# Yun-960/Pytorch-Distributed-Template

Hardware: AMD Instinct MI355X
Metric: images/sec (whole node) ResNet-50 synthetic 3x224x224 at 1/2/4/8 MI355X (higher is better)
Workload: dtype bf16; 1 GPU; model=resnet50, global_batch=2048, per_gpu_batch=2048, image_size=224, parallelism=dp1, backend=native, optimizer=SGD(lr=0.1, momentum=0.9, wd=5e-5), dist_backend=nccl, ddp=True, ddp_impl=BucketedDDP, device=cuda, hip_graph=False, ddp_fallback_copies=0

## Files before the change

### csrc/conv3x3_halo.hip

```cpp
#include "conv_nt_kernel.h"

namespace pdt_nt {
namespace {

constexpr int HBM = 224;
constexpr int HWM = 2;
constexpr int PMAX = 384;
constexpr int PBYTES = PMAX * 128;
constexpr int ZBYTES = 1024;

template <int BN, int NTH, int SGN, int BNB>
__global__ void __launch_bounds__(NTH, 1) conv3x3_halo_kernel(NTParams p, int rs_log2, int ntm, int ntn, int ncc) {
  constexpr int WN = NTH / 64 / HWM;
  constexpr int MI = HBM / (HWM * 16);
  constexpr int NI = BN / (WN * 16);
  constexpr int SB = BN * 128;
  constexpr int LB = BN * 8 / NTH;
  constexpr int GP = NTH / 8;
  constexpr int LP = PMAX / GP;
  constexpr int ZOFF = 2 * PBYTES + ZBYTES / 2;
  constexpr int SLOT0 = 2 * PBYTES + ZBYTES;
  static_assert(LB >= 1 && NI >= 1 && PMAX % GP == 0 && LB + LP <= 63, "halo tile shape");
  __shared__ __attribute__((aligned(16))) char smem[SLOT0 + 3 * SB];

  const int tid = threadIdx.x, lane = tid & 63, wave = tid >> 6;
  const int wm = wave / WN, wn = wave % WN;
  const int W = p.Ws, H = p.Hs, Cin = p.Cs, K = p.K;
  const int rs = 1 << rs_log2;
  const int k = HBM / W;
  const int P = (k + 2) * rs;
  const int NH = p.M / W;

  for (int z = tid; z < ZBYTES / 16; z += NTH)
    *reinterpret_cast<u32x4*>(smem + 2 * PBYTES + z * 16) = u32x4{0u, 0u, 0u, 0u};

  int aoff[MI][3][2];
  int lrow[MI];
#pragma unroll
  for (int i = 0; i < MI; ++i) {
    const int r = wm * (HBM / HWM) + i * 16 + (lane & 15);
    const int lr = r / W, w = r - (r / W) * W;
    lrow[i] = lr;
    const int pb = (lr + 1) * rs + w + 1;
#pragma unroll
    for (int b = 0; b < 3; ++b) {
      const int q = pb + b - 1;
#pragma unroll
      for (int kk = 0; kk < 2; ++kk) aoff[i][b][kk] = q * 128 + (((q & 7) ^ (kk * 4 + (lane >> 4))) << 4);
    }
  }
  int boff[NI][2];
#pragma unroll
  for (int j = 0; j < NI; ++j) {
    const int row = wn * (BN / WN) + j * 16 + (lane & 15);
#pragma unroll
    for (int kk = 0; kk < 2; ++kk) boff[j][kk] = row * 128 + (swz(row, kk * 4 + (lane >> 4)) << 4);
  }

  const int ntiles = ntm * ntn;
  const int my_tiles = ntiles > (int)blockIdx.x ? (ntiles - 1 - (int)blockIdx.x) / (int)gridDim.x + 1 : 0;
  const int nitems = my_tiles * ncc;
  auto item_tile = [&](int it) -> int { return (int)blockIdx.x + (it / ncc) * (int)gridDim.x; };

  auto issue_b = [&](int it, int tap, int slot) __attribute__((always_inline)) {
    const bool live = it < nitems;
    const int tile = live ? item_tile(it) : 0;
    const int n0 = (tile % ntn) * BN;
    const int cc = live ? it % ncc : 0;
    char* sb = smem + SLOT0 + slot * SB;
#pragma unroll
    for (int j = 0; j < LB; ++j) {
      const int r = (tid >> 3) + (NTH / 8) * j;
      const void* g = live ? (const void*)(p.b + (size_t)(n0 + r) * K + tap * Cin + cc * 64 + swz(r, tid & 7) * 8)
                           : p.zero;
      __builtin_amdgcn_global_load_lds(g, (__attribute__((address_space(3))) void*)(sb + (8 * wave + (NTH / 8) * j) * 128),
                                       16, 0, 0);
    }
  };
  auto issue_patch = [&](int it, int buf) __attribute__((always_inline)) {
    const bool live = it < nitems;
    const int tile = live ? item_tile(it) : 0;
    const int g0 = (tile / ntn) * k - 1;
    const int cc = live ? it % ncc : 0;
    char* sp = smem + buf * PBYTES;
#pragma unroll
    for (int l = 0; l < LP; ++l) {
      const int q = (tid >> 3) + GP * l;
      const int g = g0 + (q >> rs_log2);
      const int w = (q & (rs - 1)) - 1;
      const bool ok = live && q < P && g >= 0 && g < NH && w >= 0 && w < W;
      const int ch = (tid & 7) ^ (q & 7);
      const void* src = ok ? (const void*)(p.src + ((size_t)g * W + w) * Cin + cc * 64 + ch * 8)
                           : p.zero;
      __builtin_amdgcn_global_load_lds(src, (__attribute__((address_space(3))) void*)(sp + (8 * wave + GP * l) * 128),
                                       16, 0, 0);
    }
  };

  f32x4 acc[MI][NI];
  auto zero_acc = [&]() __attribute__((always_inline)) {
#pragma unroll
    for (int i = 0; i < MI; ++i)
#pragma unroll
      for (int j = 0; j < NI; ++j) acc[i][j] = f32x4{0.f, 0.f, 0.f, 0.f};
  };
  zero_acc();
  __syncthreads();

  if (nitems > 0) {
    issue_patch(0, 0);
    issue_b(0, 0, 0);
    issue_b(0, 1, 1);
  }
  bool after_epi = false;
  for (int it = 0; it < nitems; ++it) {
    const int tile = item_tile(it);
    const int tm = tile / ntn, tn = tile % ntn;
    const int cc = it % ncc;
    const int pbuf = it & 1;
    bool vtop[MI], vbot[MI];
#pragma unroll
    for (int i = 0; i < MI; ++i) {
      const uint32_t gr = (uint32_t)(tm * k + lrow[i]);
      const uint32_t h = gr - fdiv(gr, p.div_HWm) * (uint32_t)H;
      vtop[i] = h != 0;
      vbot[i] = h != (uint32_t)(H - 1);
    }
#pragma unroll
    for (int t = 0; t < 9; ++t) {
      if (t == 0) {
        if (after_epi) asm volatile("s_waitcnt vmcnt(0)" ::: "memory");
        else asm volatile("s_waitcnt vmcnt(%0)" ::"n"(LB) : "memory");
      } else if (t <= 2) {
        asm volatile("s_waitcnt vmcnt(%0)" ::"n"(LB + LP) : "memory");
      } else {
        asm volatile("s_waitcnt vmcnt(%0)" ::"n"(LB) : "memory");
      }
      __builtin_amdgcn_s_barrier();
      asm volatile("" ::: "memory");
      {
        const int t2 = t + 2;
        issue_b(t2 < 9 ? it : it + 1, t2 < 9 ? t2 : t2 - 9, t2 % 3);
      }
      if (t == 0) issue_patch(it + 1, pbuf ^ 1);
      const int th = t / 3, tw = t % 3;
      const int a = SGN * (th - 1), b = SGN * (tw - 1);
      const char* sb = smem + SLOT0 + (t % 3) * SB;
      const int rowoff = pbuf * PBYTES + a * rs * 128;
#pragma unroll
      for (int kk = 0; kk < 2; ++kk) {
        bf16x8 bfr[NI], af[MI];
#pragma unroll
        for (int j = 0; j < NI; ++j) bfr[j] = *reinterpret_cast<const bf16x8*>(sb + boff[j][kk]);
#pragma unroll
        for (int i = 0; i < MI; ++i) {
          int addr = aoff[i][b + 1][kk] + rowoff;
          if (a < 0 && !vtop[i]) addr = ZOFF;
          if (a > 0 && !vbot[i]) addr = ZOFF;
          af[i] = *reinterpret_cast<const bf16x8*>(smem + addr);
        }
#pragma unroll
        for (int i = 0; i < MI; ++i)
#pragma unroll
          for (int j = 0; j < NI; ++j)
            acc[i][j] = __builtin_amdgcn_mfma_f32_16x16x32_bf16(bfr[j], af[i], acc[i][j], 0, 0, 0);
      }
    }
    after_epi = false;
    if (cc != ncc - 1) continue;

    after_epi = true;
    const int m0 = tm * HBM, n0 = tn * BN;
    const int lr16 = lane & 15, lc = (lane >> 4) * 4;
    if constexpr (!BNB) {
      if (p.stats != nullptr) {
        typedef float f32x2 __attribute__((ext_vector_type(2)));
        const int srow = tm * HWM + wm;
#pragma unroll
        for (int j = 0; j < NI; ++j) {
          f32x2 s01 = {0.f, 0.f}, s23 = s01, q01 = s01, q23 = s01;
#pragma unroll
          for (int i = 0; i < MI; ++i) {
            const f32x2 v01 = {acc[i][j][0], acc[i][j][1]}, v23 = {acc[i][j][2], acc[i][j][3]};
            s01 += v01;
            s23 += v23;
            q01 = __builtin_elementwise_fma(v01, v01, q01);
            q23 = __builtin_elementwise_fma(v23, v23, q23);
          }
          float s[4] = {row16_sum(s01.x), row16_sum(s01.y), row16_sum(s23.x), row16_sum(s23.y)};
          float q[4] = {row16_sum(q01.x), row16_sum(q01.y), row16_sum(q23.x), row16_sum(q23.y)};
          if (lr16 < 8) {
            const int r = lr16 & 3;
            const float sv = (r & 2) ? ((r & 1) ? s[3] : s[2]) : ((r & 1) ? s[1] : s[0]);
            const float qv = (r & 2) ? ((r & 1) ? q[3] : q[2]) : ((r & 1) ? q[1] : q[0]);
            const int col = n0 + wn * (BN / WN) + j * 16 + lc + r;
            p.stats[(size_t)((lr16 < 4 ? 0 : p.nstat_rows) + srow) * p.Ncol + col] = lr16 < 4 ? sv : qv;
          }
        }
      }
#pragma unroll
      for (int i = 0; i < MI; ++i) {
        const int m = m0 + wm * (HBM / HWM) + i * 16 + lr16;
        if (m >= p.M) continue;
#pragma unroll
        for (int j = 0; j < NI; ++j) {
          const int col = n0 + wn * (BN / WN) + j * 16 + lc;
          typedef uint32_t u32x2 __attribute__((ext_vector_type(2)));
          *reinterpret_cast<u32x2*>(p.out + (size_t)m * p.ldo + col) =
              u32x2{pack2bf(acc[i][j][0], acc[i][j][1]), pack2bf(acc[i][j][2], acc[i][j][3])};
        }
      }
    } else {
      typedef float f32x2 __attribute__((ext_vector_type(2)));
#pragma unroll
      for (int j = 0; j < NI; ++j) {
        const int col = n0 + wn * (BN / WN) + j * 16 + lc;
        const f32x4 mu = *reinterpret_cast<const f32x4*>(p.bnb.mean + col);
        f32x4 sc = {0.f, 0.f, 0.f, 0.f}, sh = sc;
        if constexpr (BNB == 2) {
          sc = *reinterpret_cast<const f32x4*>(p.bnb.scale + col);
          sh = *reinterpret_cast<const f32x4*>(p.bnb.shift + col);
        }
        f32x2 s01 = {0.f, 0.f}, s23 = s01, q01 = s01, q23 = s01;
        uint2 yv[MI];
        uint32_t mv[MI];
#pragma unroll
        for (int i = 0; i < MI; ++i) {
          const int m = m0 + wm * (HBM / HWM) + i * 16 + lr16;
          const size_t e = (size_t)(m < p.M ? m : 0) * p.ldo + col;
          yv[i] = *reinterpret_cast<const uint2*>(p.bnb.y + e);
          mv[i] = BNB == 3 ? (uint32_t)(p.bnb.mask[e >> 3] >> (e & 7)) : 0xfu;
        }
#pragma unroll
        for (int i = 0; i < MI; ++i) {
          const int m = m0 + wm * (HBM / HWM) + i * 16 + lr16;
          const bool rok = m < p.M;
          const size_t e = (size_t)(rok ? m : 0) * p.ldo + col;
          const uint2 yy = yv[i];
          const uint32_t mk = mv[i];
          const uint32_t w0 = pack2bf(acc[i][j][0], acc[i][j][1]), w1 = pack2bf(acc[i][j][2], acc[i][j][3]);
          if (rok) {
            typedef uint32_t u32x2 __attribute__((ext_vector_type(2)));
            *reinterpret_cast<u32x2*>(p.out + e) = u32x2{w0, w1};
          }
          const uint32_t kb = rok ? mk : 0u;
          const uint32_t g0w = w0 & pdt_bf16_pair_keep(kb, 0), g1w = w1 & pdt_bf16_pair_keep(kb, 1);
          f32x2 ga = {lo_bf(g0w), hi_bf(g0w)}, gb = {lo_bf(g1w), hi_bf(g1w)};
          const f32x2 ya = {lo_bf(yy.x), hi_bf(yy.x)}, yb = {lo_bf(yy.y), hi_bf(yy.y)};
          if constexpr (BNB == 2) {
            const f32x2 za = __builtin_elementwise_fma(ya, f32x2{sc[0], sc[1]}, f32x2{sh[0], sh[1]});
            const f32x2 zb = __builtin_elementwise_fma(yb, f32x2{sc[2], sc[3]}, f32x2{sh[2], sh[3]});
            ga.x = za.x > 0.f ? ga.x : 0.f;
            ga.y = za.y > 0.f ? ga.y : 0.f;
            gb.x = zb.x > 0.f ? gb.x : 0.f;
            gb.y = zb.y > 0.f ? gb.y : 0.f;
          }
          s01 += ga;
          s23 += gb;
          q01 = __builtin_elementwise_fma(ga, ya - f32x2{mu[0], mu[1]}, q01);
          q23 = __builtin_elementwise_fma(gb, yb - f32x2{mu[2], mu[3]}, q23);
        }
        float s[4] = {s01.x, s01.y, s23.x, s23.y}, q[4] = {q01.x, q01.y, q23.x, q23.y};
#pragma unroll
        for (int r = 0; r < 4; ++r) {
          s[r] = row16_sum(s[r]);
          q[r] = row16_sum(q[r]);
        }
        if (lr16 == 0) {
          const int prow = p.bnb.row0 + tm * HWM + wm;
#pragma unroll
          for (int r = 0; r < 4; ++r) {
            p.bnb.part[(size_t)prow * p.Ncol + col + r] = s[r];
            p.bnb.part[(size_t)(p.bnb.R + prow) * p.Ncol + col + r] = q[r];
          }
        }
      }
    }
    zero_acc();
  }
  asm volatile("s_waitcnt vmcnt(0)" ::: "memory");
}

template <int BN, int NTH>
int launch_halo(const NTParams& p, int sgn, int rs_log2, hipStream_t st) {
  const int ntm = (p.M + HBM - 1) / HBM, ntn = p.Ncol / BN, ncc = p.Cs / 64;
  int grid = ntm * ntn;
  if (grid > 256) grid = 256;
  const int bnb = p.bnb.part == nullptr ? 0 : !p.bnb.relu ? 1 : p.bnb.mask == nullptr ? 2 : 3;
  auto go = [&](auto sgn_c, auto bnb_c) {
    hipLaunchKernelGGL((conv3x3_halo_kernel<BN, NTH, decltype(sgn_c)::value, decltype(bnb_c)::value>), dim3(grid),
                       dim3(NTH), 0, st, p, rs_log2, ntm, ntn, ncc);
  };
  using std::integral_constant;
  if (sgn > 0) {
    if (bnb == 0) go(integral_constant<int, 1>{}, integral_constant<int, 0>{});
    else if (bnb == 1) go(integral_constant<int, 1>{}, integral_constant<int, 1>{});
    else if (bnb == 2) go(integral_constant<int, 1>{}, integral_constant<int, 2>{});
    else go(integral_constant<int, 1>{}, integral_constant<int, 3>{});
  } else {
    if (bnb == 0) go(integral_constant<int, -1>{}, integral_constant<int, 0>{});
    else if (bnb == 1) go(integral_constant<int, -1>{}, integral_constant<int, 1>{});
    else if (bnb == 2) go(integral_constant<int, -1>{}, integral_constant<int, 2>{});
    else go(integral_constant<int, -1>{}, integral_constant<int, 3>{});
  }
  PDT_RETURN_LAUNCH();
}

constexpr int HALO_BN[NVAR_HALO] = {64, 128, 128};

}

int halo_geometry(const NTParams& p, int hv, int* sgn, int* rs_log2) {
  if (hv < 0 || hv >= NVAR_HALO) return -3;
  if (p.nth != 3 || p.ntw != 3 || p.sh != 1 || p.sw != 1 || !p.ident_out) return -5;
  if (p.Hm != p.Hs || p.Wm != p.Ws || p.pix != p.Cs || p.Cs % 64 != 0 || p.K != 9 * p.Cs || p.ldb != p.K) return -5;
  if (p.bias != nullptr || p.act != 0 || p.aux != nullptr || p.addend != nullptr || p.ldo != p.Ncol) return -5;
  if (p.Ncol % HALO_BN[hv] != 0) return -5;
  if (p.dh == 1 && p.dw == 1 && p.oh0 == -1 && p.ow0 == -1) *sgn = 1;
  else if (p.dh == -1 && p.dw == -1 && p.oh0 == 1 && p.ow0 == 1) *sgn = -1;
  else return -5;
  const int W = p.Ws;
  if (W < 1 || HBM % W != 0) return -5;
  int rs = 16, l = 4;
  while (rs < W + 2) { rs <<= 1; ++l; }
  if ((HBM / W + 2) * rs > PMAX) return -5;
  if ((long long)p.M * p.Ncol >= (1LL << 31) || (long long)p.M * p.Cs >= (1LL << 31)) return -5;
  *rs_log2 = l;
  return 0;
}

int halo_rows(int M) { return ((M + HBM - 1) / HBM) * HWM; }

int run_halo(int hv, const NTParams& p_in, hipStream_t st) {
  if (p_in.bnb.part2 != nullptr) return -5;
  int sgn = 0, rs_log2 = 0;
  const int rc = halo_geometry(p_in, hv, &sgn, &rs_log2);
  if (rc) return rc;
  NTParams p = p_in;
  p.div_HWm = make_fastdiv(p.Hs);
  p.zero = zero_chunk_addr();
  if (p.zero == nullptr) return PDT_ERR_SYMBOL;
  switch (hv) {
    case 0: return launch_halo<64, 256>(p, sgn, rs_log2, st);
    case 1: return launch_halo<128, 512>(p, sgn, rs_log2, st);
    case 2: return launch_halo<128, 256>(p, sgn, rs_log2, st);
  }
  return -3;
}

namespace {

struct HWParams {
  const u16* dy;
  const u16* x;
  float* slab;
  const void* zero;
  int M, Mo, C, H, W, rs_log2, ntiles, tps, nco, ncc;
  FastDiv div_H;
};

constexpr int HW_DY = HBM * 128;
constexpr int HW_ZOFF = 2 * PBYTES + 2 * HW_DY;
constexpr int HW_LDS = HW_ZOFF + ZBYTES;

__device__ __forceinline__ bf16x4 tr_read(const char* smem, int byte) {
  return __builtin_amdgcn_ds_read_tr16_b64_v4bf16(
      (bf16x4 __attribute__((address_space(3)))*)((__attribute__((address_space(3))) char*)(uintptr_t)(uint32_t)(
          uintptr_t)(smem + byte)));
}

__global__ void __launch_bounds__(512, 1) wgrad3x3_halo_kernel(HWParams p) {
  constexpr int NTH = 512, KS = HBM / 32;
  constexpr int LP = PMAX / (NTH / 8);
  __shared__ __attribute__((aligned(16))) char smem[HW_LDS];
  const int tid = threadIdx.x, lane = tid & 63, wave = tid >> 6;
  const int wc = wave >> 2, wg = wave & 3;
  const int W = p.W, H = p.H, C = p.C;
  const int rs = 1 << p.rs_log2;
  const int k = HBM / W;
  const int P = (k + 2) * rs;
  const int NH = p.M / W;

  const int bid = (int)blockIdx.x;
  const int ct = bid % p.nco, cc = (bid / p.nco) % p.ncc, split = bid / (p.nco * p.ncc);
  const int co0 = ct * 64;
  const int t_begin = split * p.tps;
  const int t_end = min(p.ntiles, t_begin + p.tps);

  for (int z = tid; z < ZBYTES / 16; z += NTH)
    *reinterpret_cast<u32x4*>(smem + HW_ZOFF + z * 16) = u32x4{0u, 0u, 0u, 0u};

  const int g = lane >> 4, q = (lane >> 2) & 3, pp = lane & 3;
  int xoff[KS][2][3];
  int lrow[KS][2];
#pragma unroll
  for (int ks = 0; ks < KS; ++ks)
#pragma unroll
    for (int h = 0; h < 2; ++h) {
      const int r = ks * 32 + 8 * g + q + 4 * h;
      const int lr = r / W, w = r - lr * W;
      lrow[ks][h] = lr;
      const int pb = (lr + 1) * rs + w + 1;
#pragma unroll
      for (int b = 0; b < 3; ++b) {
        const int px = pb + b - 1;
        xoff[ks][h][b] = px * 128 + ((((wg * 2 + (pp >> 1)) ^ ((px >> 1) & 7))) << 4) + (pp & 1) * 8;
      }
    }
  auto dyoff = [&](int ks, int h, int mi) -> int {
    const int r = ks * 32 + 8 * g + q + 4 * h;
    return r * 128 + (((wc * 4 + mi * 2 + (pp >> 1)) ^ ((r >> 1) & 7)) << 4) + (pp & 1) * 8;
  };

  auto issue = [&](int tj, int buf) __attribute__((always_inline)) {
    const bool live = tj < t_end;
    const int g0 = (live ? tj : 0) * k - 1;
    char* sp = smem + buf * PBYTES;
#pragma unroll
    for (int l = 0; l < LP; ++l) {
      const int qq = (tid >> 3) + (NTH / 8) * l;
      const int gr = g0 + (qq >> p.rs_log2);
      const int w = (qq & (rs - 1)) - 1;
      const bool ok = live && qq < P && gr >= 0 && gr < NH && w >= 0 && w < W;
      const int ch = (tid & 7) ^ ((qq >> 1) & 7);
      const void* src = ok ? (const void*)(p.x + ((size_t)gr * W + w) * C + cc * 64 + ch * 8)
                           : p.zero;
      __builtin_amdgcn_global_load_lds(src, (__attribute__((address_space(3))) void*)(sp + (8 * wave + 64 * l) * 128),
                                       16, 0, 0);
    }
    char* sd = smem + 2 * PBYTES + buf * HW_DY;
    const int m0 = (live ? tj : 0) * HBM;
#pragma unroll
    for (int l = 0; l < 4; ++l) {
      if (l == 3 && wave >= 4) break;
      const int r = (tid >> 3) + 64 * l;
      const int m = m0 + r;
      const int ch = (tid & 7) ^ ((r >> 1) & 7);
      const void* src = (live && m < p.M) ? (const void*)(p.dy + (size_t)m * p.Mo + co0 + ch * 8)
                                          : p.zero;
      __builtin_amdgcn_global_load_lds(src, (__attribute__((address_space(3))) void*)(sd + (8 * wave + 64 * l) * 128),
                                       16, 0, 0);
    }
  };

  f32x4 acc[9][2];
#pragma unroll
  for (int t = 0; t < 9; ++t) acc[t][0] = acc[t][1] = f32x4{0.f, 0.f, 0.f, 0.f};
  __syncthreads();

  if (t_begin < t_end) issue(t_begin, 0);
  for (int tj = t_begin; tj < t_end; ++tj) {
    const int buf = (tj - t_begin) & 1;
    asm volatile("s_waitcnt vmcnt(0)" ::: "memory");
    __builtin_amdgcn_s_barrier();
    asm volatile("" ::: "memory");
    issue(tj + 1, buf ^ 1);
    bool vt[KS][2], vb[KS][2];
#pragma unroll
    for (int ks = 0; ks < KS; ++ks)
#pragma unroll
      for (int h = 0; h < 2; ++h) {
        const uint32_t gr = (uint32_t)(tj * k + lrow[ks][h]);
        const uint32_t hh = gr - fdiv(gr, p.div_H) * (uint32_t)H;
        vt[ks][h] = hh != 0;
        vb[ks][h] = hh != (uint32_t)(H - 1);
      }
    const int pbase = buf * PBYTES;
    const int dbase = 2 * PBYTES + buf * HW_DY;
#pragma unroll
    for (int ks = 0; ks < KS; ++ks) {
      bf16x8 dyf[2];
#pragma unroll
      for (int mi = 0; mi < 2; ++mi) {
        const bf16x4 lo = tr_read(smem, dbase + dyoff(ks, 0, mi));
        const bf16x4 hi = tr_read(smem, dbase + dyoff(ks, 1, mi));
        dyf[mi] = bf16x8{lo[0], lo[1], lo[2], lo[3], hi[0], hi[1], hi[2], hi[3]};
      }
#pragma unroll
      for (int t = 0; t < 9; ++t) {
        const int a = t / 3 - 1, b = t % 3 - 1;
        int o0 = xoff[ks][0][b + 1] + pbase + a * rs * 128;
        int o1 = xoff[ks][1][b + 1] + pbase + a * rs * 128;
        if (a < 0) {
          if (!vt[ks][0]) o0 = HW_ZOFF + 256;
          if (!vt[ks][1]) o1 = HW_ZOFF + 256;
        }
        if (a > 0) {
          if (!vb[ks][0]) o0 = HW_ZOFF + 256;
          if (!vb[ks][1]) o1 = HW_ZOFF + 256;
        }
        const bf16x4 lo = tr_read(smem, o0);
        const bf16x4 hi = tr_read(smem, o1);
        const bf16x8 xf = bf16x8{lo[0], lo[1], lo[2], lo[3], hi[0], hi[1], hi[2], hi[3]};
#pragma unroll
        for (int mi = 0; mi < 2; ++mi)
          acc[t][mi] = __builtin_amdgcn_mfma_f32_16x16x32_bf16(xf, dyf[mi], acc[t][mi], 0, 0, 0);
      }
    }
  }
  asm volatile("s_waitcnt vmcnt(0)" ::: "memory");
  float* out = p.slab + (size_t)split * p.Mo * (9 * C);
#pragma unroll
  for (int t = 0; t < 9; ++t)
#pragma unroll
    for (int mi = 0; mi < 2; ++mi) {
      const int co = co0 + wc * 32 + mi * 16 + (lane & 15);
      const int c = cc * 64 + wg * 16 + (lane >> 4) * 4;
      *reinterpret_cast<f32x4*>(out + (size_t)co * (9 * C) + t * C + c) = acc[t][mi];
    }
}

}

int halo_wgrad_plan(int M, int Mo, int C, int Hs, int Ws, int* splits, int* tps) {
  if (C % 64 || Mo % 64 || Ws < 1 || HBM % Ws) return -5;
  int rs = 16;
  while (rs < Ws + 2) rs <<= 1;
  if ((HBM / Ws + 2) * rs > PMAX || (long long)M * C >= (1LL << 31) || (long long)M * Mo >= (1LL << 31)) return -5;
  const int ntiles = (M + HBM - 1) / HBM;
  const int blocks = (Mo / 64) * (C / 64);
  int s = (256 + blocks - 1) / blocks;
  if (s > ntiles) s = ntiles;
  if (s < 1) s = 1;
  const int per = (ntiles + s - 1) / s;
  *tps = per;
  *splits = (ntiles + per - 1) / per;
  return 0;
}

int run_halo_wgrad(const void* dy, const void* x, float* slab, int M, int Mo, int C, int Hs, int Ws, int splits,
                   int tps, hipStream_t st) {
  int s2 = 0, t2 = 0;
  const int rc = halo_wgrad_plan(M, Mo, C, Hs, Ws, &s2, &t2);
  if (rc) return rc;
  if (s2 != splits || t2 != tps) return -2;
  HWParams p;
  p.dy = (const u16*)dy;
  p.x = (const u16*)x;
  p.slab = slab;
  p.zero = zero_chunk_addr();
  if (p.zero == nullptr) return PDT_ERR_SYMBOL;
  p.M = M; p.Mo = Mo; p.C = C; p.H = Hs; p.W = Ws;
  int l = 4, rs = 16;
  while (rs < Ws + 2) { rs <<= 1; ++l; }
  p.rs_log2 = l;
  p.ntiles = (M + HBM - 1) / HBM;
  p.tps = tps;
  p.nco = Mo / 64;
  p.ncc = C / 64;
  p.div_H = make_fastdiv(Hs);
  hipLaunchKernelGGL(wgrad3x3_halo_kernel, dim3(p.nco * p.ncc * splits), dim3(512), 0, st, p);
  PDT_RETURN_LAUNCH();
}

}
```

### csrc/conv_nt_kernel.h

```cpp
#pragma once
#include "pdt_common.h"
#include <stdlib.h>

namespace pdt_nt {

struct BnbArgs {
  const u16* y;
  const float* mean;
  const float* scale;
  const float* shift;
  const uint8_t* mask;
  float* part;
  int relu, row0, R;
  const u16* y2 = nullptr;
  const float* mean2 = nullptr;
  float* part2 = nullptr;
};

constexpr uint32_t AX_NONE = 0xffffffffu;

struct AXArgs {
  int mode;
  int ctr;
  const u16* y2;
  const float* c1;
  const float* c2;
  const float* c3;
  const float* rsc;
  const float* rsh;
  const uint8_t* mask_in;
  uint8_t* mask_out;
  u16* dst;
};

struct NTParams {
  const u16* src;
  const u16* b;
  u16* out;
  float* stats;
  const float* bias;
  const u16* addend;
  int Hs, Ws, Cs;
  int Hm, Wm;
  int M, Ncol, K, ldb;
  int sh, sw, oh0, ow0, dh, dw, nth, ntw;
  int Ho, Wo, osh, osw, oph, opw, ldo;
  int act;
  int pix;
  u16* aux;
  int nstat_rows;
  int nt_store;
  int ident_out;
  const uint8_t* addend_mask;
  const float* dq_a;
  const float* dq_b;
  BnbArgs bnb;
  AXArgs ax;
  FastDiv div_Wm, div_HWm, div_Cs8, div_ntw;
  uint8_t* q8;
  const float* q8_meta;
  float* q8_part;
  int q8_fmt;
  int q8_only;
  const void* zero;
};

constexpr int BK = 64;
constexpr int NT = 256;

__device__ __forceinline__ float gelu_grad(float z) {
  const float u = 0.7978845608f * (z + 0.044715f * z * z * z);
  const float t = pdt_tanh(u);
  const float du = 0.7978845608f * (1.f + 3.f * 0.044715f * z * z);
  return 0.5f * (1.f + t) + 0.5f * z * (1.f - t * t) * du;
}

__device__ __forceinline__ void gelu_dual(float z, float& g, float& d) { pdt_gelu_dual(z, g, d); }

__device__ __forceinline__ int swz(int row, int chunk) { return chunk ^ ((row >> 1) & 7); }

typedef int i32x8 __attribute__((ext_vector_type(8)));
__device__ __forceinline__ i32x8 cat8(const bf16x8& lo, const bf16x8& hi) {
  const u32x4 a = __builtin_bit_cast(u32x4, lo), b = __builtin_bit_cast(u32x4, hi);
  return i32x8{(int)a[0], (int)a[1], (int)a[2], (int)a[3], (int)b[0], (int)b[1], (int)b[2], (int)b[3]};
}

static __device__ __attribute__((aligned(64))) u32x4 pdt_zero_chunk[4];
static inline const void* zero_chunk_addr() {
  static const void* cache[PDT_MAX_DEV] = {};
  return pdt_symbol_addr(HIP_SYMBOL(pdt_zero_chunk), cache);
}

template <int BM, int BN, int NSTAGE, bool CS64, bool DIRECT, bool GLDS, int NTH = 256, int WM = 2, int F8 = 0,
          int PIPE = 0, bool BNB = false, int AX = 0>
__global__ void __launch_bounds__(NTH, PIPE ? 1 : 2) conv_nt_kernel(NTParams p) {
  static_assert(AX == 0 || (!PIPE && F8 == 0 && CS64), "the A-staging BN apply: bf16, 64-channel chunks, no ring");
  constexpr int WN = NTH / 64 / WM;
  constexpr int MI = BM / (WM * 16);
  constexpr int NI = BN / (WN * 16);
  constexpr int LA = BM * 8 / NTH;
  constexpr int LB = BN * 8 / NTH;
  constexpr int RS = NTH / 8;
  constexpr int A_BYTES = BM * BK * 2;
  constexpr int B_BYTES = BN * BK * 2;
  constexpr int STAGE = A_BYTES + B_BYTES;
  constexpr int C_STRIDE = BN * 2 + 16;
  constexpr int CST = (DIRECT && !BNB) ? 0 : BM * C_STRIDE;
  constexpr int SMEM = (NSTAGE * STAGE > CST) ? NSTAGE * STAGE : CST;
  __shared__ __attribute__((aligned(16))) char smem[SMEM];

  const int tid = threadIdx.x;
  const int lane = tid & 63;
  const int wave = tid >> 6;
  const int wm = wave / WN, wn = wave % WN;
  const void* zchunk = p.zero;
  auto wcol = [&](int j) -> int {
    if constexpr (PIPE == 2)
      return j < NI / 2 ? wn * (BN / 2 / WN) + j * 16 : BN / 2 + wn * (BN / 2 / WN) + (j - NI / 2) * 16;
    else
      return wn * (BN / WN) + j * 16;
  };

  const int ntm = (p.M + BM - 1) / BM;
  const int ntn = (p.Ncol + BN - 1) / BN;
#define PDT_TILE_DONE return
#define PDT_TILE_ID blockIdx.x
#include "conv_nt_tile.inc"
#undef PDT_TILE_ID
#undef PDT_TILE_DONE
}

template <int BM, int BN, int NSTAGE, bool CS64, bool DIRECT, bool GLDS, int NTH = 256, int WM = 2, int F8 = 0,
          int PIPE = 0, bool BNB = false, int AX = 0>
__global__ void __launch_bounds__(NTH, 1) conv_nt_kernel_pers(NTParams p_arg) {
  static_assert(PIPE && AX == 0 && F8 == 0, "persistent: the bf16 1-workgroup-per-CU ring tiles");
  constexpr int WN = NTH / 64 / WM;
  constexpr int MI = BM / (WM * 16);
  constexpr int NI = BN / (WN * 16);
  constexpr int LA = BM * 8 / NTH;
  constexpr int LB = BN * 8 / NTH;
  constexpr int RS = NTH / 8;
  constexpr int A_BYTES = BM * BK * 2;
  constexpr int B_BYTES = BN * BK * 2;
  constexpr int STAGE = A_BYTES + B_BYTES;
  constexpr int C_STRIDE = BN * 2 + 16;
  constexpr int CST = (DIRECT && !BNB) ? 0 : BM * C_STRIDE;
  constexpr int SMEM = (NSTAGE * STAGE > CST) ? NSTAGE * STAGE : CST;
  __shared__ __attribute__((aligned(16))) char smem[SMEM];
  const int tid = threadIdx.x;
  const int lane = tid & 63;
  const int wave = tid >> 6;
  const int wm = wave / WN, wn = wave % WN;
  auto wcol = [&](int j) -> int {
    if constexpr (PIPE == 2)
      return j < NI / 2 ? wn * (BN / 2 / WN) + j * 16 : BN / 2 + wn * (BN / 2 / WN) + (j - NI / 2) * 16;
    else
      return wn * (BN / WN) + j * 16;
  };
  const int ntm = (p_arg.M + BM - 1) / BM;
  const int ntn = (p_arg.Ncol + BN - 1) / BN;
  const int ntiles = ntm * ntn;
  for (int tile = blockIdx.x; tile < ntiles; tile += gridDim.x) {
    if (tile != (int)blockIdx.x) __syncthreads();
    const NTParams& p = p_arg;
    const void* zchunk = p.zero;
#define PDT_TILE_DONE continue
#define PDT_TILE_ID tile
#include "conv_nt_tile.inc"
#undef PDT_TILE_ID
#undef PDT_TILE_DONE
  }
}

template <int BM, int BN, int NS, bool CS64, bool DIRECT, bool GLDS = false, int NTH = 256, int WM = 2, int F8 = 0,
          int PIPE = 0, bool BNB = false, int AX = 0, bool PERS = false>
int launch(const NTParams& p, hipStream_t st) {
  int ntm = (p.M + BM - 1) / BM, ntn = (p.Ncol + BN - 1) / BN;
  NTParams q = p;
  q.zero = zero_chunk_addr();
  if (q.zero == nullptr) return PDT_ERR_SYMBOL;
  if constexpr (PERS) {
    if (p.q8 != nullptr) return -5;
    const int grid = ntm * ntn < 256 ? ntm * ntn : 256;
    hipLaunchKernelGGL((conv_nt_kernel_pers<BM, BN, NS, CS64, DIRECT, GLDS, NTH, WM, F8, PIPE, BNB, AX>),
                       dim3(grid), dim3(NTH), 0, st, q);
  } else {
    hipLaunchKernelGGL((conv_nt_kernel<BM, BN, NS, CS64, DIRECT, GLDS, NTH, WM, F8, PIPE, BNB, AX>),
                       dim3(ntm * ntn), dim3(NTH), 0, st, q);
  }
  PDT_RETURN_LAUNCH();
}

constexpr int NVAR = 38;
constexpr int VAR_BM[NVAR] = {128, 256, 64, 128, 64, 128, 256, 64, 128, 64,
                              128, 256, 64, 128, 64, 128, 256, 64, 128, 64,
                              128, 256, 64, 128, 64, 128, 256, 64, 128, 64,
                              256, 128, 256, 128, 256, 128, 256, 256};
constexpr int VAR_BN[NVAR] = {128, 64, 128, 64, 64, 128, 64, 128, 64, 64,
                              128, 64, 128, 64, 64, 128, 64, 128, 64, 64,
                              128, 64, 128, 64, 64, 128, 64, 128, 64, 64,
                              128, 256, 128, 256, 128, 256, 256, 256};
constexpr int VAR_WM[NVAR] = {2, 2, 2, 2, 2, 2, 2, 2, 2, 2, 2, 2, 2, 2, 2, 2, 2, 2, 2, 2,
                              2, 2, 2, 2, 2, 2, 2, 2, 2, 2, 4, 2, 4, 2, 4, 2, 2, 2};

inline int heuristic_variant(int M, int Ncol, int K) {
  (void)M;
  if (Ncol <= 64) return K <= 64 ? 6 : 1;
  return K <= 64 ? 5 : 0;
}

template <bool CS64, bool BNB = false>
int launch_variant(int v, const NTParams& p, hipStream_t st) {
  switch (v) {
    case 0: return launch<128, 128, 2, CS64, false, false, 256, 2, 0, false, BNB>(p, st);
    case 1: return launch<256, 64, 2, CS64, false, false, 256, 2, 0, false, BNB>(p, st);
    case 2: return launch<64, 128, 2, CS64, false, false, 256, 2, 0, false, BNB>(p, st);
    case 3: return launch<128, 64, 2, CS64, false, false, 256, 2, 0, false, BNB>(p, st);
    case 4: return launch<64, 64, 2, CS64, false, false, 256, 2, 0, false, BNB>(p, st);
    case 5: return launch<128, 128, 1, CS64, false, false, 256, 2, 0, false, BNB>(p, st);
    case 6: return launch<256, 64, 1, CS64, false, false, 256, 2, 0, false, BNB>(p, st);
    case 7: return launch<64, 128, 1, CS64, false, false, 256, 2, 0, false, BNB>(p, st);
    case 8: return launch<128, 64, 1, CS64, false, false, 256, 2, 0, false, BNB>(p, st);
    case 9: return launch<64, 64, 1, CS64, false, false, 256, 2, 0, false, BNB>(p, st);
    case 10: return launch<128, 128, 2, CS64, true, false, 256, 2, 0, false, BNB>(p, st);
    case 11: return launch<256, 64, 2, CS64, true, false, 256, 2, 0, false, BNB>(p, st);
    case 12: return launch<64, 128, 2, CS64, true, false, 256, 2, 0, false, BNB>(p, st);
    case 13: return launch<128, 64, 2, CS64, true, false, 256, 2, 0, false, BNB>(p, st);
    case 14: return launch<64, 64, 2, CS64, true, false, 256, 2, 0, false, BNB>(p, st);
    case 15: return launch<128, 128, 1, CS64, true, false, 256, 2, 0, false, BNB>(p, st);
    case 16: return launch<256, 64, 1, CS64, true, false, 256, 2, 0, false, BNB>(p, st);
    case 17: return launch<64, 128, 1, CS64, true, false, 256, 2, 0, false, BNB>(p, st);
    case 18: return launch<128, 64, 1, CS64, true, false, 256, 2, 0, false, BNB>(p, st);
    case 19: return launch<64, 64, 1, CS64, true, false, 256, 2, 0, false, BNB>(p, st);
    case 20: return launch<128, 128, 2, CS64, false, true, 256, 2, 0, false, BNB>(p, st);
    case 21: return launch<256, 64, 2, CS64, false, true, 256, 2, 0, false, BNB>(p, st);
    case 22: return launch<64, 128, 2, CS64, false, true, 256, 2, 0, false, BNB>(p, st);
    case 23: return launch<128, 64, 2, CS64, false, true, 256, 2, 0, false, BNB>(p, st);
    case 24: return launch<64, 64, 2, CS64, false, true, 256, 2, 0, false, BNB>(p, st);
    case 25: return launch<128, 128, 1, CS64, false, true, 256, 2, 0, false, BNB>(p, st);
    case 26: return launch<256, 64, 1, CS64, false, true, 256, 2, 0, false, BNB>(p, st);
    case 27: return launch<64, 128, 1, CS64, false, true, 256, 2, 0, false, BNB>(p, st);
    case 28: return launch<128, 64, 1, CS64, false, true, 256, 2, 0, false, BNB>(p, st);
    case 29: return launch<64, 64, 1, CS64, false, true, 256, 2, 0, false, BNB>(p, st);
    case 30: return launch<256, 128, 2, CS64, false, true, 512, 4, 0, false, BNB>(p, st);
    case 31: return launch<128, 256, 2, CS64, false, true, 512, 2, 0, false, BNB>(p, st);
    case 32: return launch<256, 128, 2, CS64, false, false, 512, 4, 0, false, BNB>(p, st);
    case 33: return launch<128, 256, 2, CS64, false, false, 512, 2, 0, false, BNB>(p, st);
    case 34: return launch<256, 128, 3, CS64, false, true, 512, 4, 0, true, BNB>(p, st);
    case 35: return launch<128, 256, 3, CS64, false, true, 512, 2, 0, true, BNB>(p, st);
    case 36: return launch<256, 256, 2, CS64, false, true, 512, 2, 0, true, BNB>(p, st);
    case 37: return launch<256, 256, 2, CS64, false, true, 512, 2, 0, 2, BNB>(p, st);
  }
  return -3;
}

constexpr int NVAR_PERS = 3;
constexpr int PERS_BASE[NVAR_PERS] = {34, 35, 36};

template <bool CS64, bool BNB = false>
int launch_variant_pers(int i, const NTParams& p, hipStream_t st) {
  switch (i) {
    case 0: return launch<256, 128, 3, CS64, false, true, 512, 4, 0, true, BNB, 0, true>(p, st);
    case 1: return launch<128, 256, 3, CS64, false, true, 512, 2, 0, true, BNB, 0, true>(p, st);
    case 2:
      if constexpr (BNB) return launch<256, 256, 2, CS64, false, true, 512, 2, 0, true, BNB, 0, true>(p, st);
      else return -5;
  }
  return -3;
}


int launch_variant_bnb(int v, bool cs64, const NTParams& p, hipStream_t st);
int launch_variant_pers_bnb(int i, bool cs64, const NTParams& p, hipStream_t st);

int launch_variant_ax(int v, const NTParams& p, hipStream_t st);

constexpr int NVAR_HALO = 3;
int run_halo(int hv, const NTParams& p, hipStream_t st);
int halo_rows(int M);
int halo_wgrad_plan(int M, int Mo, int C, int Hs, int Ws, int* splits, int* tps);
int run_halo_wgrad(const void* dy, const void* x, float* slab, int M, int Mo, int C, int Hs, int Ws, int splits,
                   int tps, hipStream_t st);

}
```

### csrc/conv_wgrad.hip

```cpp
#include "pdt_common.h"
#include <stdlib.h>
#include <type_traits>

namespace pdt_nt {
int halo_wgrad_plan(int M, int Mo, int C, int Hs, int Ws, int* splits, int* tps);
int run_halo_wgrad(const void* dy, const void* x, float* slab, int M, int Mo, int C, int Hs, int Ws, int splits,
                   int tps, hipStream_t st);
}

namespace {

struct WGParams {
  const u16* dy;
  const u16* x;
  float* slab;
  int M;
  int Mo, No;
  int ldy;
  int Hs, Ws, C;
  int pix;
  int Hm, Wm;
  int sh, sw, oh0, ow0, dh, dw, ntw;
  int ktiles_per_split, splits;
  int xcd;
  float* bslab;
  const u16* bn_y;
  const float* bn_c;
  FastDiv div_Wm, div_HWm, div_C, div_ntw;
  const void* zero;
};

constexpr int BK = 64;
constexpr int NT = 256;

static __device__ __attribute__((aligned(64))) u32x4 wg_zero_chunk[4];

template <int RB>
__device__ __forceinline__ int seg_swz(int row) {
  if (RB >= 256) return (row & 3) | ((row >> 1) & 4);
  return ((row >> 1) & 1) | ((row >> 2) & 2);
}

template <int RB>
__device__ __forceinline__ int lds_off(int row, int byte_in_row) {
  int seg = byte_in_row >> 5;
  return row * RB + ((seg ^ seg_swz<RB>(row)) << 5) + (byte_in_row & 31);
}

template <int RB>
__device__ __forceinline__ bf16x8 tr_frag(const char* base, int krow0, int col0, int lane) {
  const int g = lane >> 4, q = (lane >> 2) & 3, pp = lane & 3;
  const int r1 = krow0 + 8 * g + q;
  const int cb = (col0 + 4 * pp) * 2;
  typedef __bf16 __attribute__((address_space(3))) * lptr;
  const char* a1 = base + lds_off<RB>(r1, cb);
  const char* a2 = base + lds_off<RB>(r1 + 4, cb);
  bf16x4 lo = __builtin_amdgcn_ds_read_tr16_b64_v4bf16((bf16x4 __attribute__((address_space(3)))*)(
      (__attribute__((address_space(3))) char*)(uintptr_t)(uint32_t)(uintptr_t)a1));
  bf16x4 hi = __builtin_amdgcn_ds_read_tr16_b64_v4bf16((bf16x4 __attribute__((address_space(3)))*)(
      (__attribute__((address_space(3))) char*)(uintptr_t)(uint32_t)(uintptr_t)a2));
  (void)sizeof(lptr);
  bf16x8 r;
  r[0] = lo[0]; r[1] = lo[1]; r[2] = lo[2]; r[3] = lo[3];
  r[4] = hi[0]; r[5] = hi[1]; r[6] = hi[2]; r[7] = hi[3];
  return r;
}

template <int BM, int BN, int NSTAGE, int NTH = NT, int WM = 2, int PF = 1, bool BIAS = false, bool BNA = false>
__global__ void __launch_bounds__(NTH, NTH == NT ? 2 : 1) wgrad_kernel(WGParams p) {
  static_assert(!BNA || (PF == 1 && !BIAS), "the staged BN-backward apply: single register slot, no bias");
  constexpr int WN = NTH / 64 / WM;
  constexpr int RBA = BM * 2;
  constexpr int RBB = BN * 2;
  constexpr int A_BYTES = BK * RBA;
  constexpr int B_BYTES = BK * RBB;
  constexpr int STAGE = A_BYTES + B_BYTES;
  constexpr int ACH = BM / 8;
  constexpr int AROWS = NTH / ACH;
  constexpr int NA = BK / AROWS;
  constexpr int BCH = BN / 8;
  constexpr int BROWS = NTH / BCH;
  constexpr int NB = BK / BROWS;
  constexpr int MI = BM / (WM * 16);
  constexpr int NI = BN / (WN * 16);
  static_assert(NA >= 1 && NB >= 1 && MI >= 1 && NI >= 1 && WM * WN * 64 == NTH, "wgrad tile shape");
  __shared__ __attribute__((aligned(16))) char smem[NSTAGE * STAGE];

  const int tid = threadIdx.x, lane = tid & 63, wave = tid >> 6;
  const int wm = wave / WN, wn = wave % WN;

  const int ntm = (p.Mo + BM - 1) / BM, ntn = (p.No + BN - 1) / BN;
  const int ntiles = ntm * ntn;
  const int bid = p.xcd ? (int)xcd_remap(blockIdx.x, gridDim.x) : (int)blockIdx.x;
  const int tile = bid % ntiles;
  const int split = bid / ntiles;
  const int tm = tile / ntn, tn = tile % ntn;
  const int co0 = tm * BM, tc0 = tn * BN;

  const int nk_total = (p.M + BK - 1) / BK;
  const int kt_begin = split * p.ktiles_per_split;
  const int kt_end = min(nk_total, kt_begin + p.ktiles_per_split);

  const int cA = tid % ACH, rA0 = tid / ACH;
  const int coA = co0 + cA * 8;
  const bool okA = coA < p.Mo;
  const int cB = tid % BCH, rB0 = tid / BCH;
  const int colB = tc0 + cB * 8;
  const bool okB = colB < p.No;
  int tap = fdiv(okB ? colB : 0, p.div_C);
  const int cB_ch = (okB ? colB : 0) - tap * p.C;
  const int th = fdiv(tap, p.div_ntw), tw = tap - th * p.ntw;
  const int offh = p.oh0 + p.dh * th, offw = p.ow0 + p.dw * tw;

  u32x4 ra[NA], rb[NB];
  u32x4 ry[BNA ? NA : 1];
  bool rv[BNA ? NA : 1];
  float c1[BNA ? 8 : 1], c2[BNA ? 8 : 1], c3[BNA ? 8 : 1], csc[BNA ? 8 : 1], csh[BNA ? 8 : 1];
  if constexpr (BNA) {
    const int c0 = okA ? coA : 0;
#pragma unroll
    for (int e = 0; e < 8; ++e) {
      c1[e] = p.bn_c[c0 + e];
      c2[e] = p.bn_c[p.Mo + c0 + e];
      c3[e] = p.bn_c[2 * p.Mo + c0 + e];
      csc[e] = p.bn_c[3 * p.Mo + c0 + e];
      csh[e] = p.bn_c[4 * p.Mo + c0 + e];
    }
  }
  const bool dobias = BIAS && tn == 0;
  f32x4 bacc[BIAS ? MI : 1];
#pragma unroll
  for (int i = 0; i < (BIAS ? MI : 1); ++i) bacc[i] = f32x4{0.f, 0.f, 0.f, 0.f};

  auto load_into = [&](int kt, u32x4 (&ra)[NA], u32x4 (&rb)[NB]) {
    const int k0 = kt * BK;
#pragma unroll
    for (int i = 0; i < NA; ++i) {
      int m = k0 + rA0 + AROWS * i;
      const bool ok = okA && m < p.M;
      ra[i] = *reinterpret_cast<const u32x4*>(ok ? (const void*)(p.dy + (size_t)m * p.ldy + coA) : p.zero);
      if constexpr (BNA) {
        rv[i] = ok;
        ry[i] = *reinterpret_cast<const u32x4*>(ok ? (const void*)(p.bn_y + (size_t)m * p.ldy + coA) : p.zero);
      }
    }
#pragma unroll
    for (int i = 0; i < NB; ++i) {
      int m = k0 + rB0 + BROWS * i;
      bool ok = okB && m < p.M;
      uint32_t mm = ok ? m : 0;
      uint32_t img = fdiv(mm, p.div_HWm);
      uint32_t rem = mm - img * (uint32_t)(p.Hm * p.Wm);
      uint32_t oh = fdiv(rem, p.div_Wm);
      uint32_t ow = rem - oh * p.Wm;
      int ih = (int)(oh * p.sh) + offh, iw = (int)(ow * p.sw) + offw;
      ok = ok && (unsigned)ih < (unsigned)p.Hs && (unsigned)iw < (unsigned)p.Ws;
      rb[i] = *reinterpret_cast<const u32x4*>(
          ok ? (const void*)(p.x + ((size_t)(img * p.Hs + ih) * p.Ws + iw) * p.pix + cB_ch) : p.zero);
    }
  };
  auto load_tile = [&](int kt) { load_into(kt, ra, rb); };
  auto store_from_db = [&](auto, int buf, const u32x4 (&ra)[NA], const u32x4 (&rb)[NB]) {
    char* sa = smem + buf * STAGE;
    char* sb = sa + A_BYTES;
#pragma unroll
    for (int i = 0; i < NA; ++i) {
      u32x4 v = ra[i];
      if constexpr (BNA) {
        float g[8], y[8];
#pragma unroll
        for (int e = 0; e < 4; ++e) {
          g[2 * e] = lo_bf(v[e]); g[2 * e + 1] = hi_bf(v[e]);
          y[2 * e] = lo_bf(ry[i][e]); y[2 * e + 1] = hi_bf(ry[i][e]);
        }
#pragma unroll
        for (int k = 0; k < 8; ++k) {
          g[k] = (y[k] * csc[k] + csh[k]) > 0.f ? g[k] : 0.f;
          g[k] = c1[k] * g[k] + c2[k] * y[k] + c3[k];
        }
#pragma unroll
        for (int e = 0; e < 4; ++e) v[e] = rv[i] ? pack2bf(g[2 * e], g[2 * e + 1]) : 0u;
      }
      *reinterpret_cast<u32x4*>(sa + lds_off<RBA>(rA0 + AROWS * i, cA * 16)) = v;
    }
#pragma unroll
    for (int i = 0; i < NB; ++i)
      *reinterpret_cast<u32x4*>(sb + lds_off<RBB>(rB0 + BROWS * i, cB * 16)) = rb[i];
  };

  f32x4 acc[MI][NI];
#pragma unroll
  for (int i = 0; i < MI; ++i)
#pragma unroll
    for (int j = 0; j < NI; ++j) acc[i][j] = f32x4{0.f, 0.f, 0.f, 0.f};

  auto compute = [&](auto, const char* sa) {
    const char* sb = sa + A_BYTES;
#pragma unroll
    for (int kk = 0; kk < 2; ++kk) {
      bf16x8 bfr[NI];
#pragma unroll
      for (int j = 0; j < NI; ++j) bfr[j] = tr_frag<RBB>(sb, kk * 32, wn * (BN / WN) + j * 16, lane);
#pragma unroll
      for (int i = 0; i < MI; ++i) {
        const bf16x8 af = tr_frag<RBA>(sa, kk * 32, wm * (BM / WM) + i * 16, lane);
#pragma unroll
        for (int j = 0; j < NI; ++j)
          acc[i][j] = __builtin_amdgcn_mfma_f32_16x16x32_bf16(bfr[j], af, acc[i][j], 0, 0, 0);
      }
    }
  };

  auto kloop = [&](auto db) {
  auto store_from = [&](int buf, const u32x4 (&ra)[NA], const u32x4 (&rb)[NB]) { store_from_db(db, buf, ra, rb); };
  auto store_tile = [&](int buf) { store_from(buf, ra, rb); };
  if constexpr (PF == 2) {
    static_assert(NSTAGE == 2, "deep prefetch uses the 2-stage LDS ring");
    u32x4 ra2[NA], rb2[NB];
    const int n = kt_end - kt_begin;
    if (n > 0) {
      load_into(kt_begin, ra, rb);
      store_from(0, ra, rb);
    }
    if (n > 1) load_into(kt_begin + 1, ra2, rb2);
    if (n > 2) load_into(kt_begin + 2, ra, rb);
    __syncthreads();
    for (int i = 0; i < n; i += 2) {
      compute(db, smem);
      if (i + 1 < n) store_from(1, ra2, rb2);
      __syncthreads();
      if (i + 3 < n) load_into(kt_begin + i + 3, ra2, rb2);
      if (i + 1 >= n) break;
      compute(db, smem + STAGE);
      if (i + 2 < n) store_from(0, ra, rb);
      __syncthreads();
      if (i + 4 < n) load_into(kt_begin + i + 4, ra, rb);
    }
  } else {
  if (kt_begin < kt_end) {
    load_tile(kt_begin);
    store_tile(0);
  }
  __syncthreads();
  for (int kt = kt_begin; kt < kt_end; ++kt) {
    const int cur = NSTAGE == 2 ? ((kt - kt_begin) & 1) : 0;
    if (kt + 1 < kt_end) load_tile(kt + 1);
    compute(db, smem + cur * STAGE);
    if (NSTAGE == 2) {
      if (kt + 1 < kt_end) store_tile(cur ^ 1);
      __syncthreads();
    } else if (kt + 1 < kt_end) {
      __syncthreads();
      store_tile(0);
      __syncthreads();
    }
  }
  }
  };
  kloop(std::integral_constant<bool, false>{});

  if constexpr (BIAS) {
    if (dobias) {
      constexpr int CPR = BM / 8, RPP = NTH / CPR;
      const int cc = tid % CPR, rr = tid / CPR;
      const int co = co0 + cc * 8;
      float bs[8] = {0.f, 0.f, 0.f, 0.f, 0.f, 0.f, 0.f, 0.f};
      if (co < p.Mo) {
        const int m1 = min(p.M, kt_end * BK);
        int m = kt_begin * BK + rr;
        for (; m + 3 * RPP < m1; m += 4 * RPP) {
          u32x4 v[4];
#pragma unroll
          for (int u = 0; u < 4; ++u) v[u] = *reinterpret_cast<const u32x4*>(p.dy + (size_t)(m + u * RPP) * p.ldy + co);
#pragma unroll
          for (int u = 0; u < 4; ++u)
#pragma unroll
            for (int e = 0; e < 4; ++e) {
              bs[2 * e] += lo_bf(v[u][e]);
              bs[2 * e + 1] += hi_bf(v[u][e]);
            }
        }
        for (; m < m1; m += RPP) {
          const u32x4 v = *reinterpret_cast<const u32x4*>(p.dy + (size_t)m * p.ldy + co);
#pragma unroll
          for (int e = 0; e < 4; ++e) {
            bs[2 * e] += lo_bf(v[e]);
            bs[2 * e + 1] += hi_bf(v[e]);
          }
        }
      }
      __syncthreads();
      float* red = reinterpret_cast<float*>(smem);
#pragma unroll
      for (int k = 0; k < 8; ++k) red[tid * 8 + k] = bs[k];
      __syncthreads();
      if (tid < CPR && co < p.Mo) {
        float t8[8] = {0.f, 0.f, 0.f, 0.f, 0.f, 0.f, 0.f, 0.f};
        for (int j = 0; j < RPP; ++j)
#pragma unroll
          for (int k = 0; k < 8; ++k) t8[k] += red[(j * CPR + tid) * 8 + k];
        float* bo = p.bslab + (size_t)split * p.Mo + co;
        *reinterpret_cast<f32x4*>(bo) = f32x4{t8[0], t8[1], t8[2], t8[3]};
        *reinterpret_cast<f32x4*>(bo + 4) = f32x4{t8[4], t8[5], t8[6], t8[7]};
      }
    }
  }

  float* out = p.slab + (size_t)split * p.Mo * p.No;
#pragma unroll
  for (int i = 0; i < MI; ++i) {
    int co = co0 + wm * (BM / WM) + i * 16 + (lane & 15);
#pragma unroll
    for (int j = 0; j < NI; ++j) {
      int tc = tc0 + wn * (BN / WN) + j * 16 + (lane >> 4) * 4;
      if (co < p.Mo && tc < p.No) {
        *reinterpret_cast<f32x4*>(out + (size_t)co * p.No + tc) = acc[i][j];
      }
    }
  }
}

__global__ void wgrad_reduce1_kernel(const float* __restrict__ slab, float* __restrict__ dst, long n4, int splits,
                                     int G, float scale, int accumulate, int final_stage) {
  long i = (long)blockIdx.x * blockDim.x + threadIdx.x;
  if (i >= n4) return;
  const int g = blockIdx.y;
  const f32x4* s = reinterpret_cast<const f32x4*>(slab) + i;
  f32x4 a = {0.f, 0.f, 0.f, 0.f}, b = {0.f, 0.f, 0.f, 0.f};
  int k = g;
  for (; k + G < splits; k += 2 * G) {
    a += s[(long)k * n4];
    b += s[(long)(k + G) * n4];
  }
  if (k < splits) a += s[(long)k * n4];
  a += b;
  f32x4* o = reinterpret_cast<f32x4*>(dst) + (final_stage ? i : (long)g * n4 + i);
  if (final_stage) {
    a *= scale;
    if (accumulate) a += *o;
  }
  *o = a;
}

}

struct WGVar {
  int BM, BN, NS, NTH, target;
};
constexpr int WG_NVAR = 28;
constexpr WGVar WG_VARS[WG_NVAR] = {
    {64, 64, 2, 256, 1024},   {64, 64, 1, 256, 1024},   {64, 64, 1, 256, 2048},
    {64, 128, 2, 256, 1024},  {64, 128, 1, 256, 1024},  {64, 128, 1, 256, 2048},
    {128, 64, 2, 256, 1024},  {128, 64, 1, 256, 1024},  {128, 64, 1, 256, 2048},
    {128, 128, 2, 256, 1024}, {128, 128, 1, 256, 1024}, {128, 128, 1, 256, 2048},
    {256, 128, 2, 512, 512},  {128, 256, 2, 512, 512},  {256, 128, 2, 512, 1024},
    {128, 256, 2, 512, 1024}, {256, 256, 2, 512, 256},  {256, 256, 2, 512, 512},
    {64, 128, 3, 256, 1024},  {128, 64, 3, 256, 1024},  {128, 128, 3, 256, 1024},
    {128, 128, 3, 256, 2048}, {64, 64, 3, 256, 2048},   {256, 128, 3, 512, 512},
    {128, 256, 3, 512, 512},  {256, 128, 3, 512, 1024}, {128, 256, 3, 512, 1024},
    {256, 256, 3, 512, 512},
};
static WGVar wg_variant(int v, int Mo, int No) {
  if (v < 0 || v >= WG_NVAR) return WGVar{Mo <= 64 ? 64 : 128, No <= 64 ? 64 : 128, 2, 256, 1024};
  return WG_VARS[v];
}

constexpr int WG_RING = WG_NVAR + 1;
PDT_API int pdt_wgrad_num_variants() { return WG_NVAR + 2; }
PDT_API int pdt_wgrad_halo_id() { return WG_NVAR; }

static int wgrad_ring_plan(int M, int Mo, int No, int* ktiles_per_split) {
  const int tiles = (Mo / 256) * (No / 256);
  const int nk = (M + BK - 1) / BK;
  const long slots = pdt_num_cus();
  int splits = 1;
  long best_cost = -1;
  for (int s = 1; s <= nk; ++s) {
    const int kps = (nk + s - 1) / s;
    if (s > 1 && kps < 8) break;
    const int se = (nk + kps - 1) / kps;
    const long cost = (((long)tiles * se + slots - 1) / slots) * kps;
    if (best_cost < 0 || cost < best_cost) {
      best_cost = cost;
      splits = s;
    }
  }
  const int kps = (nk + splits - 1) / splits;
  *ktiles_per_split = kps;
  return (nk + kps - 1) / kps;
}

static void launch_wg_bna(const WGVar& w, dim3 grid, const WGParams& p, hipStream_t stream) {
#define WG_LAUNCH_B(a, b, c) hipLaunchKernelGGL((wgrad_kernel<a, b, c, NT, 2, 1, false, true>), grid, dim3(NT), 0, stream, p)
  if (w.NS == 2) {
    if (w.BM == 64 && w.BN == 64) WG_LAUNCH_B(64, 64, 2);
    else if (w.BM == 64) WG_LAUNCH_B(64, 128, 2);
    else if (w.BN == 64) WG_LAUNCH_B(128, 64, 2);
    else WG_LAUNCH_B(128, 128, 2);
  } else {
    if (w.BM == 64 && w.BN == 64) WG_LAUNCH_B(64, 64, 1);
    else if (w.BM == 64) WG_LAUNCH_B(64, 128, 1);
    else if (w.BN == 64) WG_LAUNCH_B(128, 64, 1);
    else WG_LAUNCH_B(128, 128, 1);
  }
#undef WG_LAUNCH_B
}

template <bool BIAS>
static void launch_wg(const WGVar& w, dim3 grid, const WGParams& p, hipStream_t stream) {
  const int BM = w.BM, BN = w.BN, NS = w.NS;
#define WG_LAUNCH(a, b, c) hipLaunchKernelGGL((wgrad_kernel<a, b, c, NT, 2, 1, BIAS>), grid, dim3(NT), 0, stream, p)
#define WG_LAUNCH8(a, b, wm) hipLaunchKernelGGL((wgrad_kernel<a, b, 2, 512, wm, 1, BIAS>), grid, dim3(512), 0, stream, p)
#define WG_LAUNCH_PF(a, b, t, wm) hipLaunchKernelGGL((wgrad_kernel<a, b, 2, t, wm, 2, BIAS>), grid, dim3(t), 0, stream, p)
  if (NS == 3) {
    if (w.NTH == 512) {
      if (BM == 256 && BN == 256) WG_LAUNCH_PF(256, 256, 512, 2);
      else if (BM == 256) WG_LAUNCH_PF(256, 128, 512, 4);
      else WG_LAUNCH_PF(128, 256, 512, 2);
    } else {
      if (BM == 64 && BN == 64) WG_LAUNCH_PF(64, 64, 256, 2);
      else if (BM == 64) WG_LAUNCH_PF(64, 128, 256, 2);
      else if (BN == 64) WG_LAUNCH_PF(128, 64, 256, 2);
      else WG_LAUNCH_PF(128, 128, 256, 2);
    }
  } else if (w.NTH == 512) {
    if (BM == 256 && BN == 256) WG_LAUNCH8(256, 256, 2);
    else if (BM == 256) WG_LAUNCH8(256, 128, 4);
    else WG_LAUNCH8(128, 256, 2);
  } else if (NS == 2) {
    if (BM == 64 && BN == 64) WG_LAUNCH(64, 64, 2);
    else if (BM == 64) WG_LAUNCH(64, 128, 2);
    else if (BN == 64) WG_LAUNCH(128, 64, 2);
    else WG_LAUNCH(128, 128, 2);
  } else {
    if (BM == 64 && BN == 64) WG_LAUNCH(64, 64, 1);
    else if (BM == 64) WG_LAUNCH(64, 128, 1);
    else if (BN == 64) WG_LAUNCH(128, 64, 1);
    else WG_LAUNCH(128, 128, 1);
  }
#undef WG_LAUNCH
#undef WG_LAUNCH8
#undef WG_LAUNCH_PF
}

template <bool BIAS, bool BNA>
static const void* wg_kernel(const WGVar& w) {
#define KP(a, b, c, t, wm, pf) return reinterpret_cast<const void*>(&wgrad_kernel<a, b, c, t, wm, pf, BIAS, BNA>)
  const int BM = w.BM, BN = w.BN, NS = w.NS;
  if constexpr (!BNA) {
    if (NS == 3) {
      if (w.NTH == 512) {
        if (BM == 256 && BN == 256) KP(256, 256, 2, 512, 2, 2);
        if (BM == 256) KP(256, 128, 2, 512, 4, 2);
        KP(128, 256, 2, 512, 2, 2);
      }
      if (BM == 64 && BN == 64) KP(64, 64, 2, NT, 2, 2);
      if (BM == 64) KP(64, 128, 2, NT, 2, 2);
      if (BN == 64) KP(128, 64, 2, NT, 2, 2);
      KP(128, 128, 2, NT, 2, 2);
    }
    if (w.NTH == 512) {
      if (BM == 256 && BN == 256) KP(256, 256, 2, 512, 2, 1);
      if (BM == 256) KP(256, 128, 2, 512, 4, 1);
      KP(128, 256, 2, 512, 2, 1);
    }
  }
  if (NS == 2) {
    if (BM == 64 && BN == 64) KP(64, 64, 2, NT, 2, 1);
    if (BM == 64) KP(64, 128, 2, NT, 2, 1);
    if (BN == 64) KP(128, 64, 2, NT, 2, 1);
    KP(128, 128, 2, NT, 2, 1);
  }
  if (BM == 64 && BN == 64) KP(64, 64, 1, NT, 2, 1);
  if (BM == 64) KP(64, 128, 1, NT, 2, 1);
  if (BN == 64) KP(128, 64, 1, NT, 2, 1);
  KP(128, 128, 1, NT, 2, 1);
#undef KP
}

static long wg_slots(int v, const WGVar& w) {
  static int cache[WG_NVAR] = {};
  if (v < 0 || v >= WG_NVAR) return 2L * pdt_num_cus();
  if (cache[v] == 0) {
    int n = 1 << 20;
    const void* ks[3] = {wg_kernel<false, false>(w), wg_kernel<true, false>(w),
                         (w.NS <= 2 && w.NTH == NT) ? wg_kernel<false, true>(w) : nullptr};
    for (const void* k : ks) {
      int b = 0;
      if (k == nullptr) continue;
      if (hipOccupancyMaxActiveBlocksPerMultiprocessor(&b, k, w.NTH, 0) != hipSuccess) b = 1;
      n = b < n ? b : n;
    }
    cache[v] = n < 1 ? 1 : n;
  }
  return (long)cache[v] * pdt_num_cus();
}

static int wgrad_plan(int M, int Mo, int No, int variant, int* ktiles_per_split) {
  const WGVar w = wg_variant(variant, Mo, No);
  const int BM = w.BM, BN = w.BN, target = w.target;
  int tiles = ((Mo + BM - 1) / BM) * ((No + BN - 1) / BN);
  int nk = (M + BK - 1) / BK;
  int smax = (target + tiles - 1) / tiles;
  if (smax > nk) smax = nk;
  if (smax < 1) smax = 1;
  static const int mode = !pdt_env_flag("PDT_WG_PLAN", 1) ? 0 : pdt_env_flag("PDT_WG_PLAN", 0) ? 1 : 2;
  int splits = smax;
  const long slots = wg_slots(variant, w);
  if (mode == 0 || (mode == 2 && slots > pdt_num_cus())) {
    while (splits > 1 && (nk + splits - 1) / splits < 8) --splits;
  } else {
    long best_cost = -1;
    for (int s = 1; s <= smax; ++s) {
      const int kps = (nk + s - 1) / s;
      if (s > 1 && kps < 8) break;
      const int se = (nk + kps - 1) / kps;
      const long cost = (((long)tiles * se + slots - 1) / slots) * kps;
      if (best_cost < 0 || cost < best_cost) {
        best_cost = cost;
        splits = s;
      }
    }
  }
  int kps = (nk + splits - 1) / splits;
  splits = (nk + kps - 1) / kps;
  *ktiles_per_split = kps;
  return splits;
}

PDT_API int pdt_wgrad_plan2(int M, int Mo, int No, int Hs, int Ws, int C, int variant, int* per_split) {
  if (variant == WG_NVAR) {
    int splits = 0;
    const int rc = pdt_nt::halo_wgrad_plan(M, Mo, C, Hs, Ws, &splits, per_split);
    return rc ? rc : splits;
  }
  if (variant == WG_RING) {
    if (pdt_wgrad_ring_ok(Mo, No, C, 0) != 0) return -5;
    return wgrad_ring_plan(M, Mo, No, per_split);
  }
  return wgrad_plan(M, Mo, No, variant, per_split);
}

static int reduce_groups(int splits, int Mo, int No) {
  long n4 = (long)Mo * No / 4;
  int xb = (int)((n4 + 255) / 256);
  int G = splits < 2 ? 1 : (int)(1024 / xb);
  if (G > splits / 4) G = splits / 4;
  if (G < 1) G = 1;
  return G;
}

PDT_API long pdt_wgrad_workspace(int splits, int Mo, int No) {
  const long G = reduce_groups(splits, Mo, No);
  return (long)splits * Mo * No + (G > 1 ? G * Mo * No : 0) + (long)splits * Mo;
}

PDT_API int pdt_conv_wgrad2(const void* dy, const void* x, float* slab, float* out, int M, int Mo, int No,
                            int ldy, int Hs, int Ws, int C, int Hm, int Wm, int sh, int sw, int oh0, int ow0,
                            int dh, int dw, int ntw, int splits, int ktiles_per_split, float scale,
                            int accumulate, int variant, int pix, float* bias_out, const void* bn_y,
                            const float* bn_c, hipStream_t stream) {
  if (C % 8 != 0 || Mo % 8 != 0 || No % 8 != 0 || ldy % 8 != 0) return -1;
  const bool bna = bn_y != nullptr;
  if (bna && (bn_c == nullptr || variant < 0 || variant >= 12 || bias_out != nullptr)) return -5;
  if (pix != 0 && (pix % 4 != 0 || pix > C)) return -10;
  if (variant == WG_NVAR) {
    if (ntw != 3 || No != 9 * C || sh != 1 || sw != 1 || oh0 != -1 || ow0 != -1 || dh != 1 || dw != 1 ||
        Hm != Hs || Wm != Ws || (pix != 0 && pix != C) || ldy != Mo || bias_out != nullptr || M % Wm != 0)
      return -5;
    const int rc = pdt_nt::run_halo_wgrad(dy, x, slab, M, Mo, C, Hs, Ws, splits, ktiles_per_split, stream);
    if (rc) return rc;
    return pdt_wgrad_reduce(slab, out, nullptr, nullptr, splits, Mo, No, scale, accumulate, stream);
  }
  if (variant == WG_RING) {
    if (bna || bias_out != nullptr) return -5;
    const int rc = pdt_wgrad_ring_launch(dy, x, slab, M, Mo, No, ldy, Hs, Ws, C, Hm, Wm, sh, sw, oh0, ow0, dh, dw, ntw,
                                         splits, ktiles_per_split, pix, stream);
    if (rc) return rc;
    return pdt_wgrad_reduce(slab, out, nullptr, nullptr, splits, Mo, No, scale, accumulate, stream);
  }
  WGParams p;
  p.dy = (const u16*)dy;
  p.x = (const u16*)x;
  p.slab = slab;
  p.M = M; p.Mo = Mo; p.No = No; p.ldy = ldy;
  p.Hs = Hs; p.Ws = Ws; p.C = C; p.Hm = Hm; p.Wm = Wm;
  p.pix = pix > 0 ? pix : C;
  p.sh = sh; p.sw = sw; p.oh0 = oh0; p.ow0 = ow0; p.dh = dh; p.dw = dw; p.ntw = ntw;
  p.ktiles_per_split = ktiles_per_split; p.splits = splits;
  p.bn_y = (const u16*)bn_y;
  p.bn_c = bn_c;
  const int G = reduce_groups(splits, Mo, No);
  p.bslab = bias_out ? slab + (long)splits * Mo * No + (G > 1 ? (long)G * Mo * No : 0) : nullptr;
  static const int xcd_env = pdt_env_flag("PDT_WGRAD_XCD", 1);
  p.xcd = xcd_env;
  p.div_Wm = make_fastdiv(Wm);
  p.div_HWm = make_fastdiv(Hm * Wm);
  p.div_C = make_fastdiv(C);
  p.div_ntw = make_fastdiv(ntw);
  {
    static const void* zc[PDT_MAX_DEV] = {};
    p.zero = pdt_symbol_addr(HIP_SYMBOL(wg_zero_chunk), zc);
    if (p.zero == nullptr) return PDT_ERR_SYMBOL;
  }
  const WGVar w = wg_variant(variant, Mo, No);
  int tiles = ((Mo + w.BM - 1) / w.BM) * ((No + w.BN - 1) / w.BN);
  dim3 grid(tiles * splits);
  if (bna) launch_wg_bna(w, grid, p, stream);
  else if (bias_out) launch_wg<true>(w, grid, p, stream);
  else launch_wg<false>(w, grid, p, stream);
  int e = (int)hipGetLastError();
  if (e) return e;
  return pdt_wgrad_reduce(slab, out, p.bslab, bias_out, splits, Mo, No, scale, accumulate, stream);
}

static int reduce_rows_groups(int nrows) {
  if (nrows <= 32) return 0;
  int G = 1;
  while (G * G < nrows) ++G;
  return G > 64 ? 64 : G;
}

PDT_API long pdt_reduce_rows_work(int nrows, int n) { return (long)reduce_rows_groups(nrows) * n; }

PDT_API int pdt_wgrad_reduce_rows(const float* rows, float* out, int nrows, int n, float scale, int accumulate,
                                  float* work, hipStream_t stream) {
  if (n % 4 != 0 || nrows < 1) return -1;
  const long n4 = n / 4;
  const int xb = (int)((n4 + 255) / 256);
  const int G = reduce_rows_groups(nrows);
  if (G > 1 && work != nullptr) {
    hipLaunchKernelGGL(wgrad_reduce1_kernel, dim3(xb, G), dim3(256), 0, stream, rows, work, n4, nrows, G, 1.f, 0, 0);
    hipLaunchKernelGGL(wgrad_reduce1_kernel, dim3(xb, 1), dim3(256), 0, stream, work, out, n4, G, 1, scale,
                       accumulate, 1);
  } else {
    hipLaunchKernelGGL(wgrad_reduce1_kernel, dim3(xb, 1), dim3(256), 0, stream, rows, out, n4, nrows, 1, scale,
                       accumulate, 1);
  }
  PDT_RETURN_LAUNCH();
}

PDT_API int pdt_wgrad_reduce(float* slab, float* out, const float* bslab, float* bias_out, int splits, int Mo, int No,
                             float scale, int accumulate, hipStream_t stream) {
  const int G = reduce_groups(splits, Mo, No);
  long n4 = (long)Mo * No / 4;
  int xb = (int)((n4 + 255) / 256);
  if (bias_out) {
    hipLaunchKernelGGL(wgrad_reduce1_kernel, dim3((Mo / 4 + 255) / 256, 1), dim3(256), 0, stream, bslab, bias_out,
                       (long)(Mo / 4), splits, 1, scale, accumulate, 1);
  }
  if (G == 1) {
    hipLaunchKernelGGL(wgrad_reduce1_kernel, dim3(xb, 1), dim3(256), 0, stream, slab, out, n4, splits, 1, scale,
                       accumulate, 1);
  } else {
    float* part = slab + (long)splits * Mo * No;
    hipLaunchKernelGGL(wgrad_reduce1_kernel, dim3(xb, G), dim3(256), 0, stream, slab, part, n4, splits, G, 1.f, 0,
                       0);
    hipLaunchKernelGGL(wgrad_reduce1_kernel, dim3(xb, 1), dim3(256), 0, stream, part, out, n4, G, 1, scale,
                       accumulate, 1);
  }
  PDT_RETURN_LAUNCH();
}
```

### csrc/pdt_api.h

```cpp
#pragma once
#include <hip/hip_runtime.h>
#include <stdint.h>

#define PDT_API extern "C" __attribute__((visibility("default")))

PDT_API int pdt_attn_set_bwd_single(int on);
PDT_API int pdt_attn_set_tiled(int on);
PDT_API int pdt_attn_fwd(const void* qkv, void* out, float* lse, int B, int T, int H, float scale, hipStream_t st);
PDT_API int pdt_attn_bwd(const void* qkv, const void* out, const void* dout, const float* lse, float* delta,
                         void* dqkv, int B, int T, int H, float scale, hipStream_t st);
PDT_API int pdt_attn_bwd_q8(const void* qkv, const void* out, const void* dout, const float* lse, float* delta,
                            void* dqkv, int B, int T, int H, float scale, void* q8, float* q8_meta, float* q8_part,
                            float* q8_dq, hipStream_t st);

PDT_API int pdt_attn_bwd_f8_grid(int B, int H);
PDT_API int pdt_attn_bwd_f8_q8(const void* qkv, const void* out, const void* dout, const float* lse, void* dqkv,
                               int B, int T, int H, float scale, void* q8, const float* q8_meta, float* q8_part,
                               float* q8_dq, float* colpart, float* bias_out, hipStream_t st);
PDT_API int pdt_attn_bwd_f8(const void* qkv, const void* out, const void* dout, const float* lse, void* dqkv, int B,
                            int T, int H, float scale, hipStream_t st);
PDT_API int pdt_attn_bwd_f8_debug(const void* qkv, const void* out, const void* dout, const float* lse, void* dqkv,
                                  int B, int T, int H, float scale, float* dbg, hipStream_t st);

PDT_API int pdt_cls_attn_fwd(const void* qkv, void* o, float* lse, int B, int T, int H, hipStream_t st);
PDT_API int pdt_cls_attn_bwd(const void* qkv, const void* o, const void* dout, const float* lse, void* dqkv, int B,
                             int T, int H, hipStream_t st);

PDT_API int pdt_attn_set_pv8(int on);
PDT_API int pdt_attn_fwd_f8(const void* qkv, void* out, float* lse, int B, int T, int H, float scale, hipStream_t st);
PDT_API int pdt_attn_fwd_f8_q8(const void* qkv, void* out, float* lse, int B, int T, int H, float scale, void* q8,
                               float* q8_meta, float* q8_part, float* q8_dq, hipStream_t st);
PDT_API int pdt_attn_fwd_tiles(const void* qkv, void* out, float* lse, int B, int T, int H, float scale,
                               hipStream_t st);

PDT_API int pdt_bn_stats_blocks(long M, int C);
PDT_API long pdt_rows_reduce_workspace(int R, int C);
PDT_API int pdt_bn_finalize(const float* part, int R, int C, double count, float eps, float momentum,
                            const float* gamma, const float* beta, float* mean, float* invstd, float* scale,
                            float* shift, float* running_mean, float* running_var, long* num_batches_tracked,
                            hipStream_t st);
PDT_API int pdt_bn_apply(const void* y, const void* res, void* out, const float* scale, const float* shift, long M,
                         int C, int relu, void* mask, hipStream_t st);
PDT_API int pdt_bn_apply_res_affine(const void* y, const void* r, void* out, const float* scale, const float* shift,
                                    const float* rscale, const float* rshift, long M, int C, int relu, void* mask,
                                    hipStream_t st);
PDT_API int pdt_bn_bwd_reduce(const void* dA, const void* y, const void* act, const float* mean, const float* scale,
                              const float* shift, float* part, long M, int C, int relu, int blocks, const void* mask,
                              hipStream_t st);
PDT_API int pdt_bn_bwd_finalize(const float* part, int R, int C, double count, const float* gamma, const float* mean,
                                const float* invstd, float* dgamma, float* dbeta, float* k1, float* k2, float* k3,
                                int accumulate, hipStream_t st);
PDT_API int pdt_bn_bwd_apply_dual(const void* dA, const void* mask, const void* y1, const float* k1a,
                                  const float* k2a, const float* k3a, void* dy1, const void* y2, const float* k1b,
                                  const float* k2b, const float* k3b, void* dy2, long M, int C, hipStream_t st);
PDT_API int pdt_bn_bwd_apply(const void* dA, const void* y, const void* act, const float* scale, const float* shift,
                             const float* k1, const float* k2, const float* k3, void* dy, void* dres, long M, int C,
                             int relu, const void* mask, hipStream_t st);
PDT_API int pdt_bn_bwd_reduce_pool(const void* dout, const void* idx, const void* y, const float* mean,
                                   const float* scale, const float* shift, float* part, int N, int H, int W, int C,
                                   int Ho, int Wo, int k, int s, int p, int blocks, hipStream_t st);
PDT_API int pdt_bn_bwd_apply_pool(const void* dout, const void* idx, const void* y, const float* scale,
                                  const float* shift, const float* k1, const float* k2, const float* k3, void* dy,
                                  int N, int H, int W, int C, int Ho, int Wo, int k, int s, int p, hipStream_t st);

PDT_API int pdt_conv_nt_num_variants();
PDT_API int pdt_conv_nt_variant_kind(int v);
PDT_API int pdt_conv_nt_resolve_variant(int variant, int M, int Ncol, int K);
PDT_API int pdt_conv_nt_bnb_rows(int M, int Ncol, int K, int variant);
PDT_API int pdt_conv_nt_bnb_supports(int variant, int has_addend, int has_mask, int relu, int two);
PDT_API int pdt_conv_nt_stat_rows(int M, int Ncol, int K, int variant);
PDT_API int pdt_conv_nt(const void* src, const void* b, void* out, float* stats, const float* bias,
                        const void* addend, const void* addend_mask, int Hs, int Ws, int Cs, int Nimg, int Hm, int Wm,
                        int Ncol, int K, int ldb, int sh, int sw, int oh0, int ow0, int dh, int dw, int nth, int ntw,
                        int Ho, int Wo, int osh, int osw, int oph, int opw, int ldo, int act, void* aux, int variant,
                        int pix, hipStream_t stream);
PDT_API int pdt_conv_nt_bnb(const void* src, const void* b, void* out, const void* addend, const void* addend_mask,
                            int Hs, int Ws, int Cs, int Nimg, int Hm, int Wm, int Ncol, int K, int ldb, int sh,
                            int sw, int oh0, int ow0, int dh, int dw, int nth, int ntw, int Ho, int Wo, int osh,
                            int osw, int oph, int opw, int ldo, int variant, const void* bn_y, const float* bn_mean,
                            const float* bn_scale, const float* bn_shift, const void* bn_mask, float* part, int relu,
                            int row0, int R, hipStream_t stream);
PDT_API int pdt_conv_nt_bnb2(const void* src, const void* b, void* out, const void* addend, const void* addend_mask,
                             int Hs, int Ws, int Cs, int Nimg, int Hm, int Wm, int Ncol, int K, int ldb, int sh,
                             int sw, int oh0, int ow0, int dh, int dw, int nth, int ntw, int Ho, int Wo, int osh,
                             int osw, int oph, int opw, int ldo, int variant, const void* bn_y, const float* bn_mean,
                             const float* bn_scale, const float* bn_shift, const void* bn_mask, float* part, int relu,
                             int row0, int R, const void* bn_y2, const float* bn_mean2, float* part2,
                             hipStream_t stream);
PDT_API int pdt_conv_nt_ax3(const void* src, const void* b, void* out, float* stats, const void* addend,
                            const void* addend_mask, int Hs, int Ws, int Cs, int Nimg, int Hm, int Wm, int Ncol,
                            int K, int ldb, int sh, int sw, int oh0, int ow0, int dh, int dw, int nth, int ntw,
                            int Ho, int Wo, int osh, int osw, int oph, int opw, int ldo, int variant,
                            const void* bn_y, const float* bn_mean, const float* bn_scale, const float* bn_shift,
                            const void* bn_mask, float* part, int relu, int row0, int R, int ax_mode,
                            const void* ax_y2, const float* ax_c1, const float* ax_c2, const float* ax_c3,
                            const float* ax_rsc, const float* ax_rsh, const void* ax_mask_in, void* ax_mask_out,
                            void* ax_dst, hipStream_t stream);
PDT_API int pdt_conv_nt_ax(const void* src, const void* b, void* out, float* stats, int Hs, int Ws, int Cs, int Nimg,
                           int Hm, int Wm, int Ncol, int K, int ldb, int ldo, int variant, const void* bn_y,
                           const float* bn_mean, const float* bn_scale, const float* bn_shift, const void* bn_mask,
                           float* part, int relu, int row0, int R, int ax_mode, const void* ax_y2, const float* ax_c1,
                           const float* ax_c2, const float* ax_c3, const float* ax_rsc, const float* ax_rsh,
                           const void* ax_mask_in, void* ax_mask_out, void* ax_dst, hipStream_t stream);
PDT_API int pdt_gemm_f8_num_variants();
PDT_API int pdt_gemm_f8(const void* a, const void* b, void* out, const float* bias, const float* dq_a,
                        const float* dq_b, int M, int N, int K, int lda, int ldb, int ldo, int fmt_a, int act,
                        void* aux, const void* addend, int variant, hipStream_t stream);
PDT_API int pdt_gemm_f8_bm(int variant);
PDT_API long pdt_gemm_f8_q8_part(int M, int N);
PDT_API int pdt_gemm_f8_q8(const void* a, const void* b, void* out, const float* bias, const float* dq_a,
                           const float* dq_b, int M, int N, int K, int lda, int ldb, int ldo, int fmt_a, int act,
                           void* aux, const void* addend, int variant, void* q8, float* q8_meta, float* q8_part,
                           int q8_fmt, int q8_only, float* q8_dq, hipStream_t stream);
PDT_API int pdt_gemm_f8_q8_cs(const void* a, const void* b, void* out, const float* bias, const float* dq_a,
                              const float* dq_b, int M, int N, int K, int lda, int ldb, int ldo, int fmt_a, int act,
                              void* aux, const void* addend, int variant, void* q8, float* q8_meta, float* q8_part,
                              int q8_fmt, int q8_only, float* q8_dq, float* colsum, hipStream_t stream);

PDT_API int pdt_wgrad_num_variants();
PDT_API int pdt_wgrad_halo_id();
PDT_API int pdt_wgrad_plan2(int M, int Mo, int No, int Hs, int Ws, int C, int variant, int* per_split);
PDT_API long pdt_wgrad_workspace(int splits, int Mo, int No);
PDT_API int pdt_conv_wgrad2(const void* dy, const void* x, float* slab, float* out, int M, int Mo, int No, int ldy,
                            int Hs, int Ws, int C, int Hm, int Wm, int sh, int sw, int oh0, int ow0, int dh, int dw,
                            int ntw, int splits, int ktiles_per_split, float scale, int accumulate, int variant,
                            int pix, float* bias_out, const void* bn_y, const float* bn_c, hipStream_t stream);
PDT_API long pdt_reduce_rows_work(int nrows, int n);
PDT_API int pdt_wgrad_reduce_rows(const float* rows, float* out, int nrows, int n, float scale, int accumulate,
                                  float* work, hipStream_t stream);
PDT_API int pdt_wgrad_reduce(float* slab, float* out, const float* bslab, float* bias_out, int splits, int Mo, int No,
                             float scale, int accumulate, hipStream_t stream);

PDT_API int pdt_drop_path_scales(float* scale, int* state, const float* p, const float* inv_keep, int n_branches,
                                 int B, long sample0, hipStream_t st);

PDT_API int pdt_ema_update(const void* chunks, int nchunks, void* ema, const void* src, void* shadows, float* dev,
                           float decay, int warmup, hipStream_t st);

PDT_API int pdt_amax_blocks(long n);
PDT_API int pdt_amax_partial(const void* x, int bf16, long n, float* partial, hipStream_t st);
PDT_API int pdt_cast_fp8(const void* x, int bf16, long n, const float* partial, int fmt, void* q, float* dq,
                         hipStream_t st);
PDT_API int pdt_cast_fp8_dual(const float* x, int R, int C, const float* partial, void* q, void* qt, float* dq,
                              hipStream_t st);
PDT_API int pdt_fp8_meta_words();
PDT_API int pdt_cast_fp8_delayed(const void* x, int bf16, long n, float* meta, int fmt, void* q, float* dq_out,
                                 hipStream_t st);
PDT_API int pdt_gelu_dual_cast_fp8(const void* y, long n, float* meta, int fmt, void* q, void* aux, void* a_out,
                                   float* dq_out, hipStream_t st);
PDT_API int pdt_cast_cs_bands(int rows);
PDT_API int pdt_cast_fp8_delayed_cs(const void* x, int rows, int cols, float* meta, int fmt, void* q, float* dq_out,
                                    float* cpart, float* bias_out, hipStream_t st);
PDT_API int pdt_cast_fp8_gelu_grad_cs(const void* x, const void* z, int rows, int cols, float* meta, int fmt, void* q,
                                      float* dq_out, float* cpart, float* bias_out, hipStream_t st);
PDT_API int pdt_fp8_meta_roll_partial(float* meta, const float* partial, int nblk, int fmt, float* dq_out,
                                      hipStream_t st);
PDT_API int pdt_fp8_meta_seed(const float* partial, long n, int fmt, float* meta, hipStream_t st);

PDT_API int pdt_gemm_ring_num_variants();
PDT_API int pdt_gemm_ring_grid(int M, int N, int sub);
PDT_API int pdt_gemm_ring_bm();
PDT_API int pdt_gemm_ring(const void* a, const void* b, void* c, const float* bias, const float* dq_a,
                          const float* dq_b, int M, int N, int K, int lda, int ldb, int ldc, int dt, int sub,
                          hipStream_t st);
PDT_API int pdt_gemm_ring_epi(const void* a, const void* b, void* c, const float* bias, const float* dq_a,
                              const float* dq_b, int M, int N, int K, int lda, int ldb, int ldc, int dt, int act,
                              void* aux, const void* addend, void* q8, const float* q8_meta, float* q8_part,
                              int q8_fmt, int q8_only, float* colsum, hipStream_t st);
PDT_API int pdt_gemm_ring_epi_pers(const void* a, const void* b, void* c, const float* bias, const float* dq_a,
                                   const float* dq_b, int M, int N, int K, int lda, int ldb, int ldc, int dt, int act,
                                   void* aux, const void* addend, void* q8, const float* q8_meta, float* q8_part,
                                   int q8_fmt, int q8_only, float* colsum, hipStream_t st);

PDT_API int pdt_crop_resize_norm_u8_bf16(const void* src, int Hs, int Ws, const int64_t* idx, const int* box,
                                         void* out, long B, int S, int Cp, const float* mean, const float* inv_std,
                                         hipStream_t st);
PDT_API int pdt_crop_resize_norm_mix_u8_bf16(const void* src, int Hs, int Ws, const int64_t* idx, const int* box,
                                             const int64_t* pidx, const int* pbox, const int* rect,
                                             const float* w_own, void* out, long B, int S, int Cp, const float* mean,
                                             const float* inv_std, hipStream_t st);
PDT_API int pdt_crop_resize_norm_erase_u8_bf16(const void* src, int Hs, int Ws, const int64_t* idx, const int* box,
                                               const int64_t* pidx, const int* pbox, const int* rect,
                                               const float* w_own, const int* erect, int R, const void* ekey,
                                               int emode, void* out, long B, int S, int Cp, const float* mean,
                                               const float* inv_std, hipStream_t st);

PDT_API int pdt_ln_fwd(const void* x, const float* g, const float* b, void* y, float* mean, float* rstd, int rows,
                       int D, float eps, hipStream_t st);
PDT_API int pdt_ln_fwd_f8_blocks(int rows);
PDT_API int pdt_ln_add_fwd(const void* x, const void* r, void* xsum, const float* g, const float* b, void* y,
                           float* mean, float* rstd, int rows, int D, float eps, void* q, float* meta,
                           float* amax_part, float* dq_out, hipStream_t st);
PDT_API int pdt_ln_add_dp_fwd(const void* x, const void* r, void* xsum, const float* g, const float* b, void* y,
                              float* mean, float* rstd, int rows, int D, float eps, void* q, float* meta,
                              float* amax_part, float* dq_out, const float* scale, int rows_per_sample,
                              hipStream_t st);
PDT_API int pdt_ln_fwd_f8(const void* x, const float* g, const float* b, void* y, float* mean, float* rstd, int rows,
                          int D, float eps, void* q, float* meta, float* amax_part, float* dq_out, hipStream_t st);
PDT_API int pdt_ln_bwd_blocks(int rows);
PDT_API int pdt_ln_bwd(const void* dy, const void* x, const float* g, const float* mean, const float* rstd, void* dx,
                       float* dg, float* db, float* part, int rows, int D, int accumulate, const void* addend,
                       hipStream_t st);
PDT_API int pdt_ln_bwd_f8(const void* dy, const void* x, const float* g, const float* mean, const float* rstd,
                          void* dx, float* dg, float* db, float* part, int rows, int D, int accumulate,
                          const void* addend, void* q8, float* q8_meta, float* q8_part, float* q8_dq, hipStream_t st);
PDT_API int pdt_ln_bwd_f8_db(const void* dy, const void* x, const float* g, const float* mean, const float* rstd,
                             void* dx, float* dg, float* db, float* part, int rows, int D, int accumulate,
                             const void* addend, void* q8, float* q8_meta, float* q8_part, float* q8_dq, float* cpart,
                             float* bias_out, int bias_acc, hipStream_t st);
PDT_API int pdt_ln_dp_bwd(const void* dy, const void* x, const float* g, const float* mean, const float* rstd,
                          void* dx, void* dyb, float* dg, float* db, float* part, int rows, int D, int accumulate,
                          const void* addend, const float* scale, int rows_per_sample, void* q8, float* q8_meta,
                          float* q8_part, float* q8_dq, float* cpart, float* bias_out, int bias_acc,
                          hipStream_t st);
PDT_API int pdt_gelu_bwd(const void* dy, const void* z, void* dz, long n, hipStream_t st);

PDT_API int pdt_lenet_grad_row(int nc);
PDT_API int pdt_lenet_fwd(const float* x, const float* w1, const float* b1, const float* w2, const float* b2,
                          const float* wf1, const float* bf1, const float* wf2, const float* bf2, int B, int NC,
                          int training, float p2, float p1, unsigned seed, float* logp, void* mask2, void* mask1,
                          hipStream_t st);
PDT_API int pdt_lenet_bwd(const float* x, const float* w1, const float* b1, const float* w2, const float* b2,
                          const float* wf1, const float* bf1, const float* wf2, const float* bf2, int B, int NC,
                          int training, float p2, float p1, unsigned seed, const float* dlogp, float* part,
                          float* grads, hipStream_t st);
PDT_API int pdt_nll_fwd(const float* logp, const int64_t* tgt, int B, int C, int ignore, float* loss, float* count,
                        float* bad, hipStream_t st);
PDT_API int pdt_nll_bwd(const int64_t* tgt, const float* g, const float* count, int B, int C, int ignore,
                        float* dlogp, hipStream_t st);

PDT_API int pdt_fill_uniform_bf16(void* out, long n, unsigned seed, hipStream_t st);
PDT_API int pdt_synth_images_bf16(void* out, const int64_t* idx, long B, int HW, int C, int Cp, unsigned seed,
                                  int64_t* labels, int classes, hipStream_t st);
PDT_API int pdt_cast_f32_bf16(const float* x, void* y, long n, hipStream_t st);
PDT_API int pdt_wt_dgrad(const float* w, void* out, int Cout, int KH, int KW, int Cin, int kh0, int kw0, int s,
                         int nth, int ntw, hipStream_t st);
PDT_API int pdt_wt_job_size();
PDT_API int pdt_wt_dgrad_multi(const void* jobs, int njobs, long total, hipStream_t st);
PDT_API int pdt_transpose_cast(const float* w, void* out, int R, int C, hipStream_t st);
PDT_API int pdt_lane_reduce_probe(const float* x, float* out, int n, hipStream_t st);

PDT_API int pdt_chunk_struct_size();
PDT_API int pdt_sgd_step2(const void* chunks, int nchunks, void* params, const void* grads, void* bufs, void* shadows,
                          float lr, float momentum, float dampening, float wd, int nesterov, int first,
                          float grad_scale, const float* dev, hipStream_t st);
PDT_API int pdt_adam_step2(const void* chunks, int nchunks, void* params, const void* grads, void* exp_avg,
                           void* exp_avg_sq, void* max_sq, void* shadows, float lr, float b1, float b2, float eps,
                           float wd, int decoupled, float bc1, float bc2, float grad_scale, float* dev, int tick,
                           hipStream_t st);

PDT_API int pdt_sumsq_chunks(const void* chunks, int nchunks, const void* a, const void* b, float* partials,
                             hipStream_t st);
PDT_API int pdt_norm_finalize(const float* partials, const int* chunk_begin, int n_tensors, int nroles, int grole,
                              float* norms, float* glob, int start_zero, float max_grad_norm, hipStream_t st);
PDT_API int pdt_lars_step(const void* chunks, int nchunks, void* params, const void* grads, void* bufs, void* shadows,
                          const int* flags, const float* norms, int n_tensors, const float* glob, float lr,
                          float momentum, float wd, int nesterov, float trust, float eps, const float* dev,
                          hipStream_t st);
PDT_API int pdt_lamb_tick(float* dev, double b1, double b2, hipStream_t st);
PDT_API int pdt_lamb_stage1(const void* chunks, int nchunks, const void* params, const void* grads, void* exp_avg,
                            void* exp_avg_sq, const int* flags, float* partials, const float* glob, float b1,
                            float b2, float omb1, float omb2, float eps, float wd, float bc1, float bc2,
                            const float* dev, hipStream_t st);
PDT_API int pdt_lamb_stage2(const void* chunks, int nchunks, void* params, const void* exp_avg,
                            const void* exp_avg_sq, void* shadows, const int* flags, const float* norms,
                            int n_tensors, float lr, float eps, float wd, float bc1, float bc2, const float* dev,
                            hipStream_t st);

PDT_API int pdt_maxpool_fwd(const void* x, void* y, void* idx, int N, int H, int W, int C, int Ho, int Wo, int k,
                            int s, int p, hipStream_t st);
PDT_API int pdt_maxpool_fwd_affine(const void* x, void* y, void* idx, const float* scale, const float* shift, int N,
                                   int H, int W, int C, int Ho, int Wo, int k, int s, int p, hipStream_t st);
PDT_API int pdt_maxpool_bwd(const void* dy, const void* idx, void* dx, int N, int H, int W, int C, int Ho, int Wo,
                            int k, int s, int p, hipStream_t st);
PDT_API int pdt_avgpool_fwd(const void* x, void* y, int N, int HW, int C, hipStream_t st);
PDT_API int pdt_avgpool_bwd(const void* dy, void* dx, int N, int HW, int C, hipStream_t st);
PDT_API int pdt_maxpool_bwd_bnred(const void* dy, const void* idx, void* dx, const void* y, const float* mean,
                                  const float* scale, const float* shift, float* part, int N, int H, int W, int C,
                                  int Ho, int Wo, int blocks, hipStream_t st);

PDT_API int pdt_stem_fwd_rows(int N, int H, int W, int Cout);
PDT_API int pdt_stem_fwd(const void* x4, const void* w256, void* y, float* part, int N, int H, int W, int Cout,
                         hipStream_t stream);
PDT_API int pdt_stem_wgrad_splits_v(int N, int H, int W, int Cout, int variant);
PDT_API int pdt_stem_wgrad_v(const void* x4, const void* dA, const void* y, const float* bnc, float* slab, int N,
                             int H, int W, int Cout, int variant, hipStream_t stream);

PDT_API int pdt_wgrad_f8_num_variants();
PDT_API int pdt_wgrad_f8_plan(int M, int Mo, int No, int variant, int* ktiles_per_split);
PDT_API long pdt_wgrad_f8_workspace(int splits, int Mo, int No);
PDT_API int pdt_linear_wgrad_f8(const void* dy8, const void* x8, const float* dq_dy, const float* dq_x,
                                const void* dy16, float* slab, float* out, float* bias_out, int M, int Mo, int No,
                                int ldy, int ldx, int splits, int ktiles_per_split, int accumulate, int variant,
                                hipStream_t stream);

PDT_API int pdt_wgrad_ring_ok(int Mo, int No, int C, int pix);
PDT_API int pdt_wgrad_ring_launch(const void* dy, const void* x, float* slab, int M, int Mo, int No, int ldy, int Hs,
                                  int Ws, int C, int Hm, int Wm, int sh, int sw, int oh0, int ow0, int dh, int dw,
                                  int ntw, int splits, int ktiles_per_split, int pix, hipStream_t st);

PDT_API int pdt_xent_fwd(const void* logits, int bf16, const long* target, float* lse, float* loss_rows,
                         float* loss_out, int B, int V, float eps, hipStream_t st);
PDT_API int pdt_xent_bwd(const void* logits, int bf16, const long* target, const float* lse, const float* gout,
                         void* dlogits, int B, int V, float eps, hipStream_t st);
PDT_API int pdt_xent_pair_fwd(const void* logits, int bf16, const long* ta, const long* tb, const float* lam,
                              float* lse, float* loss_rows, float* loss_out, int B, int V, float eps,
                              hipStream_t st);
PDT_API int pdt_xent_pair_bwd(const void* logits, int bf16, const long* ta, const long* tb, const float* lam,
                              const float* lse, const float* gout, void* dlogits, int B, int V, float eps,
                              hipStream_t st);
PDT_API long pdt_colsum_workspace(int R, int C);
PDT_API int pdt_colsum(const void* x, float* out, float* work, int R, int C, int acc, hipStream_t st);
```

### pytorch_distributed_template_amd/ops/autotune.py

```python
from __future__ import annotations

import contextlib
import json
import os
from functools import lru_cache
from pathlib import Path

import torch

NOT_APPLICABLE = -5
AX_UNFUSED = -2

SHIPPED_PATH = (Path(os.environ["PDT_LIB_PATH"]).parent if os.environ.get("PDT_LIB_PATH")
                else Path(__file__).resolve().parents[1] / "_lib") / "autotune_gfx950.json"
CACHE_PATH = Path(os.environ.get("PDT_AUTOTUNE_CACHE", str(Path.home() / ".cache" / "pytorch_distributed_template_amd"
                                                           / "autotune_gfx950.json")))
_table: dict | None = None
_forced = _frozen = False
_retuned: set = set()
_RETUNE = {"PDT_RETUNE_WITH": ("PDT_RETUNE_PREFIX", True), "PDT_RETUNE_WG": (None, True),
           "PDT_RETUNE_AX": (None, False)}


def tuned() -> dict:
    global _table
    if _table is None:
        _table = {}
        paths = (SHIPPED_PATH, CACHE_PATH) if os.environ.get("PDT_AUTOTUNE_SHIPPED", "1") != "0" else (CACHE_PATH,)
        for path in paths:
            try:
                _table.update(json.loads(Path(path).read_text()))
            except Exception:
                pass
    return _table


def save():
    if os.environ.get("RANK", "0") != "0" or CACHE_PATH.resolve() == SHIPPED_PATH.resolve():
        return
    try:
        CACHE_PATH.parent.mkdir(parents=True, exist_ok=True)
        tmp = str(CACHE_PATH) + f".tmp{os.getpid()}"
        Path(tmp).write_text(json.dumps(_table, indent=0, sort_keys=True))
        os.replace(tmp, CACHE_PATH)
    except Exception:
        pass


def capturing() -> bool:
    return torch.cuda.is_available() and torch.cuda.is_current_stream_capturing()


def tune_allowed() -> bool:
    if _frozen or capturing():
        return False
    if os.environ.get("PDT_AUTOTUNE", "1") == "0" or os.environ.get("PDT_DETERMINISTIC", "0") == "1":
        return False
    return _forced or int(os.environ.get("WORLD_SIZE", "1")) <= 1


@contextlib.contextmanager
def forced_tuning():
    global _forced
    _forced = True
    try:
        yield
    finally:
        _forced = False


def adopt(table: dict) -> None:
    global _frozen
    tuned().clear()
    _table.update(table)
    _frozen = True


def trial_ms(fn) -> float:
    ev0, ev1 = torch.cuda.Event(enable_timing=True), torch.cuda.Event(enable_timing=True)
    ev0.record()
    for _ in range(3):
        fn()
    ev1.record()
    ev1.synchronize()
    return ev0.elapsed_time(ev1)


def time_candidates(ids, launch, rounds) -> dict:
    best = {}
    for v in ids:
        rc = launch(v)
        if rc == NOT_APPLICABLE:
            continue
        if rc:
            raise RuntimeError(f"tune variant {v} failed with code {rc}")
        best[v] = float("inf")
    for _ in range(rounds):
        for v in best:
            best[v] = min(best[v], trial_ms(lambda: launch(v)))
    return best


def _ms(fn) -> float:
    return time_candidates((0,), lambda _: fn() and 0, 2)[0]


def id_set(spec) -> set:
    out = set()
    for part in spec.split(","):
        lo, _, hi = part.partition("-")
        out.update(range(int(lo), int(hi or lo) + 1))
    return out


def _retune_ids(key, table, var):
    spec = os.environ.get(var)
    if not spec or key in _retuned or key not in table or not tune_allowed():
        return None
    prefix = _RETUNE[var][0]
    if prefix and not key.startswith(os.environ.get(prefix, "")):
        return None
    _retuned.add(key)
    return id_set(spec) | {int(table[key])}


def choose(key, setup, default, *, retune=None, first_only=None, ref=None, ref_value=AX_UNFUSED, ref_first=False):
    table = tuned()
    ids = _retune_ids(key, table, retune) if retune else None
    if ids is None and key in table:
        return int(table[key])
    if not tune_allowed():
        return default() if callable(default) else default
    cand, launch = setup()
    if ids is None:
        spec = os.environ.get(first_only) if first_only else None
        ids = id_set(spec) if spec else None
    elif not _RETUNE[retune][1]:
        cand, ids = sorted(v for v in ids if v >= 0), None
    if ids is not None:
        cand = [v for v in cand if v in ids]
    times = time_candidates(cand, launch, max(1, int(os.environ.get("PDT_TUNE_ROUNDS", "2"))))
    best = min(times, key=times.get) if times else -1
    if ref is not None:
        if ref_first:
            ref()
        if best >= 0 and _ms(ref) < _ms(lambda: launch(best)):
            best = ref_value
    table[key] = best
    save()
    return best


def _csv(*xs) -> str:
    return ",".join(str(x) for x in xs)


@lru_cache(maxsize=None)
def nt_key(Hs, Ws, Cs, Nimg, Hm, Wm, Ncol, K, sh, sw, nth, ntw, osh, with_stats, has_bias, pix=0, act=0) -> str:
    return "nt5:" + _csv(Hs, Ws, Cs, Nimg, Hm, Wm, Ncol, K, sh, sw, nth, ntw, osh, int(with_stats), int(has_bias)) + \
        (f",p{pix}" if pix else "") + (f",a{int(act)}" if act else "")


@lru_cache(maxsize=None)
def ntb_key(Hs, Ws, Cs, Nimg, Hm, Wm, Ncol, K, sh, sw, nth, ntw, osh, has_addend, has_mask, two=False) -> str:
    return "ntb2:" + _csv(Hs, Ws, Cs, Nimg, Hm, Wm, Ncol, K, sh, sw, nth, ntw, osh, int(has_addend), int(has_mask)) + \
        (",2" if two else "")


@lru_cache(maxsize=None)
def wg_key(M, Mo, No, Hs, Ws, C, Hm, Wm, sh, ntw, pix=0, bn=False) -> str:
    return ("wgb:" if bn else "wg2:") + _csv(M, Mo, No, Hs, Ws, C, Hm, Wm, sh, ntw) + (f",p{pix}" if pix else "")


@lru_cache(maxsize=None)
def axf_key(H, W, Cs, N, Cout, has_res, has_ru, with_stats, KH=1, KW=1, ph=0) -> str:
    return "axf:" + _csv(H, W, Cs, N, Cout, int(has_res), int(has_ru), int(with_stats)) + \
        (f",k{KH}x{KW}p{ph}" if KH != 1 or KW != 1 else "")


def axb_key(H, W, Cout, N, Cin, side=False) -> str:
    return ("axd:" if side else "axb:") + _csv(H, W, Cout, N, Cin)


@lru_cache(maxsize=None)
def ax3_key(Ho, Wo, Cout, N, Cin, KH, KW, ph, has_addend=False, has_addend_mask=False, has_bnb_mask=False) -> str:
    return "ax3:" + _csv(Ho, Wo, Cout, N, Cin, KH, KW, ph) + \
        (f",a{int(has_addend)}{int(has_addend_mask)}m{int(has_bnb_mask)}" if has_addend or has_bnb_mask else "")


def stem_key(N, H, W, Cout, wgrad=False) -> str:
    return ("stem2w:" if wgrad else "stem1:") + _csv(N, H, W, Cout)


@lru_cache(maxsize=None)
def f8_key(M, N, K, fmt_a, act, has_bias, residual=False, q8=None, colsum=False) -> str:
    return "f8c:" + _csv(M, N, K, fmt_a, act, int(has_bias)) + (",r" if residual else "") + \
        (f",q{q8[0]}{int(q8[1])}" if q8 is not None else "") + (",cs" if colsum else "")


@lru_cache(maxsize=None)
def wg8_key(M, Nout, K) -> str:
    return "wg8:" + _csv(M, Nout, K)
```

### pytorch_distributed_template_amd/ops/native_ops/bn_unit.py

```python
from __future__ import annotations

import os

import torch
import torch.nn as nn

from .. import autotune
from .conv import (_BnbPartials, _DGRAD_W, _conv_dgrad, _conv_forward, _conv_wgrad, _fwd_geom, _fwd_nt_geom,
                   supports_conv)
from .gemm import _AX_MAX_ELEMS, _check_addend
from .lib import _chk, _cl, _empty_cl, _grad_buf, _load, _p, _s, fallback
from .shadows import bf16_weight
from .tuning import NOT_APPLICABLE


class _BNArgs:
    __slots__ = ("training", "momentum", "eps", "rm", "rv", "nbt")

    def __init__(self, bn: nn.BatchNorm2d):
        self.training = bn.training or not bn.track_running_stats
        self.momentum = bn.momentum if bn.momentum is not None else 0.1
        self.eps = bn.eps
        self.rm = bn.running_mean if (bn.track_running_stats and bn.training) else None
        self.rv = bn.running_var if (bn.track_running_stats and bn.training) else None
        self.nbt = None
        if bn.training and bn.track_running_stats and bn.num_batches_tracked is not None:
            self.nbt = bn.num_batches_tracked
            if bn.momentum is None:
                self.nbt.add_(1)
                self.momentum = 1.0 / float(self.nbt.item())
                self.nbt = None
        if not self.training:
            self.rm, self.rv = bn.running_mean, bn.running_var


class _Unit:
    __slots__ = ("x", "w", "gamma", "beta", "y", "act", "mask", "mean", "invstd", "scale", "shift", "N", "C", "Cs", "H",
                 "W", "Cout", "g", "relu", "has_res", "bnb_pre", "pend", "res_unit", "__weakref__")


def nhwc_padded_view(x, cp):
    if getattr(x, "pdt_nhwc_pad", None) != cp or x.dtype != torch.bfloat16 or x.dim() != 4:
        return None
    N, C, H, W = x.shape
    if x.stride() != (H * W * cp, 1, W * cp, cp):
        return None
    if x.untyped_storage().nbytes() < (x.storage_offset() + N * H * W * cp) * 2:
        return None
    return torch.as_strided(x, (N, cp, H, W), (H * W * cp, 1, W * cp, cp))


def _unit_fwd(x, w, gamma, beta, residual, conv, relu, bna: _BNArgs, apply: bool = True, res_unit=None,
              src_pend=None, defer: bool = False):
    lib = _load()
    st = _s()
    N, C, H, W = x.shape
    Cs = C if C % 8 == 0 else 8
    xp = nhwc_padded_view(x, Cs) if Cs != C else None
    x = x.to(torch.bfloat16)
    if xp is not None:
        x = xp
    elif Cs != C:
        x = torch.nn.functional.pad(_cl(x).permute(0, 2, 3, 1), (0, Cs - C)).permute(0, 3, 1, 2)
    x = _cl(x)
    Cout = w.shape[0]
    g = _fwd_geom(N, H, W, Cs, conv)
    wb = bf16_weight(w, pad_cin_to=Cs if Cs != C else None)
    f32 = dict(dtype=torch.float32, device=x.device)
    M = N * g["Ho"] * g["Wo"]
    r = None
    if src_pend is not None and getattr(src_pend, "pend", None) is not None:
        assert src_pend.y.shape == x.shape and x.data_ptr() == src_pend.pend[2].data_ptr()
        r = _conv_fwd_ax(src_pend, x, wb, N, H, W, Cs, Cout, g, bna.training)
        if r is None:
            _materialize(src_pend)
        src_pend.pend = None
    if r is None:
        r = _conv_forward(x, wb, N, H, W, Cs, Cout, g, with_stats=bna.training)
    y, _, part, R = r
    if bna.training:
        vec = torch.empty((4, Cout), **f32)
        mean, invstd, scale, shift = vec[0], vec[1], vec[2], vec[3]
        _chk(lib.pdt_bn_finalize(_p(part), R, Cout, float(M), float(bna.eps), float(bna.momentum), _p(gamma),
                                 _p(beta), _p(mean), _p(invstd), _p(scale), _p(shift), _p(bna.rm), _p(bna.rv),
                                 _p(bna.nbt), st), "bn_finalize")
    else:
        invstd = torch.rsqrt(bna.rv.float() + bna.eps)
        mean = bna.rm.float().clone()
        scale = (gamma.float() * invstd).contiguous()
        shift = (beta.float() - mean * scale).contiguous()
    assert y.numel() == M * Cout
    if not apply:
        u = _Unit()
        u.x, u.w, u.gamma, u.beta, u.y = x, w, gamma, beta, y
        u.act, u.mask, u.bnb_pre, u.pend, u.res_unit = None, None, None, None, None
        u.mean, u.invstd, u.scale, u.shift = mean, invstd, scale, shift
        u.N, u.C, u.Cs, u.H, u.W, u.Cout, u.g, u.relu, u.has_res = N, C, Cs, H, W, Cout, g, relu, False
        return None, u
    res = None
    if residual is not None:
        res = _cl(residual)
        assert res.dtype == torch.bfloat16 and res.shape == y.shape, (res.shape, y.shape)
    out = torch.empty_like(y, memory_format=torch.channels_last)
    mask = torch.empty(M * Cout // 8, dtype=torch.uint8, device=x.device) if (relu and residual is not None) \
        else None
    if res_unit is not None:
        assert residual is res_unit.y and res_unit.Cout == Cout
    u = _Unit()
    u.pend = None
    if defer and relu:
        u.pend = (res, res_unit, out)
    elif res_unit is not None:
        _chk(lib.pdt_bn_apply_res_affine(_p(y), _p(res), _p(out), _p(scale), _p(shift), _p(res_unit.scale),
                                         _p(res_unit.shift), M, Cout, int(relu), _p(mask), st), "bn_apply_res_affine")
    else:
        _chk(lib.pdt_bn_apply(_p(y), _p(res), _p(out), _p(scale), _p(shift), M, Cout, int(relu), _p(mask), st),
             "bn_apply")
    u.x, u.w, u.gamma, u.beta, u.y = x, w, gamma, beta, y
    u.act = None
    u.mask = mask
    u.res_unit = res_unit
    u.bnb_pre = None
    u.mean, u.invstd, u.scale, u.shift = mean, invstd, scale, shift
    u.N, u.C, u.Cs, u.H, u.W, u.Cout, u.g, u.relu, u.has_res = N, C, Cs, H, W, Cout, g, relu, residual is not None
    return out, u


def _bn_bwd(dA, u: _Unit, want_dres: bool, mask=None, pre: _BnbPartials | None = None, coeffs_only=False):
    lib = _load()
    st = _s()
    dA = _cl(dA.to(torch.bfloat16))
    Cout = u.Cout
    M = u.N * u.g["Ho"] * u.g["Wo"]
    f32 = dict(dtype=torch.float32, device=dA.device)
    if mask is None:
        mask = u.mask
    relu = u.relu or mask is not None
    if pre is not None:
        assert pre.unit is u
        part, blocks = pre.part, pre.R
    else:
        blocks = lib.pdt_bn_stats_blocks(M, Cout)
        part = torch.empty(2 * blocks * Cout + lib.pdt_rows_reduce_workspace(blocks, Cout), **f32)
        _chk(lib.pdt_bn_bwd_reduce(_p(dA), _p(u.y), _p(u.act), _p(u.mean), _p(u.scale), _p(u.shift), _p(part), M,
                                   Cout, int(relu), blocks, _p(mask), st), "bn_bwd_reduce")
    vec = torch.empty((3, Cout), **f32)
    k1, k2, k3 = vec[0], vec[1], vec[2]
    dgamma, dbeta = _grad_buf(u.gamma, (Cout,)), _grad_buf(u.beta, (Cout,))
    _chk(lib.pdt_bn_bwd_finalize(_p(part), blocks, Cout, float(M), _p(u.gamma), _p(u.mean), _p(u.invstd),
                                 _p(dgamma), _p(dbeta), _p(k1), _p(k2), _p(k3), 0, st), "bn_bwd_finalize")
    if coeffs_only:
        return dgamma, dbeta, k1, k2, k3
    dy = torch.empty_like(u.y, memory_format=torch.channels_last)
    dres = torch.empty_like(u.y, memory_format=torch.channels_last) if want_dres else None
    _chk(lib.pdt_bn_bwd_apply(_p(dA), _p(u.y), _p(u.act), _p(u.scale), _p(u.shift), _p(k1), _p(k2), _p(k3),
                              _p(dy), _p(dres), M, Cout, int(relu), _p(mask), st), "bn_bwd_apply")
    return dy, dres, dgamma, dbeta


def _bn_bwd_pool(dout, idx, u: _Unit, k, s, p):
    lib = _load()
    st = _s()
    N, C, H, W = u.N, u.Cout, u.g["Ho"], u.g["Wo"]
    Ho, Wo = dout.shape[2], dout.shape[3]
    assert dout.is_contiguous(memory_format=torch.channels_last) and dout.dtype == torch.bfloat16
    assert idx.numel() == N * Ho * Wo * C and u.y.shape == (N, C, H, W)
    assert u.relu and u.act is None and u.mask is None
    M = N * H * W
    f32 = dict(dtype=torch.float32, device=dout.device)
    rp = 256 // (C // 8)
    blocks = max(1, min(int(os.environ.get("PDT_POOL_BN_BLOCKS", "4096")), (M + rp - 1) // rp))
    part = torch.empty(2 * blocks * C + lib.pdt_rows_reduce_workspace(blocks, C), **f32)
    _chk(lib.pdt_bn_bwd_reduce_pool(_p(dout), _p(idx), _p(u.y), _p(u.mean), _p(u.scale), _p(u.shift), _p(part),
                                    N, H, W, C, Ho, Wo, k, s, p, blocks, st), "bn_bwd_reduce_pool")
    vec = torch.empty((3, C), **f32)
    k1, k2, k3 = vec[0], vec[1], vec[2]
    dgamma, dbeta = _grad_buf(u.gamma, (C,)), _grad_buf(u.beta, (C,))
    _chk(lib.pdt_bn_bwd_finalize(_p(part), blocks, C, float(M), _p(u.gamma), _p(u.mean), _p(u.invstd),
                                 _p(dgamma), _p(dbeta), _p(k1), _p(k2), _p(k3), 0, st), "bn_bwd_finalize")
    dy = torch.empty_like(u.y, memory_format=torch.channels_last)
    _chk(lib.pdt_bn_bwd_apply_pool(_p(dout), _p(idx), _p(u.y), _p(u.scale), _p(u.shift), _p(k1), _p(k2), _p(k3),
                                   _p(dy), N, H, W, C, Ho, Wo, k, s, p, st), "bn_bwd_apply_pool")
    return dy, dgamma, dbeta


def _unit_dx(dy, u: _Unit, addend=None, addend_mask=None, bnb_unit=None, bnb_mask=None, bnb_unit2=None):
    wd = u.w
    if u.Cs != u.C:
        wd = torch.nn.functional.pad(u.w.detach().float(), (0, 0, 0, 0, 0, u.Cs - u.C))
        assert addend is None and bnb_unit is None
    dx = _conv_dgrad(dy, wd, u.N, u.H, u.W, u.Cs, u.Cout, u.g, addend=addend, addend_mask=addend_mask,
                     bnb_unit=bnb_unit, bnb_mask=bnb_mask, bnb_unit2=bnb_unit2)
    return dx[:, :u.C] if u.Cs != u.C else dx


AX_VARIANTS = (0, 1, 3, 5, 6, 8, 10, 13, 15, 16, 18, 20, 23, 25, 26, 28, 30, 31)


def _ax_enabled() -> bool:
    return os.environ.get("PDT_FUSE_BN_AX", "1") != "0"


def _conv1_fold_enabled() -> bool:
    return os.environ.get("PDT_FUSE_BN_AX1", "1") != "0"


_NO_BNB = (None, None, None, None, None, None, 0, 0, 0)


def _ax_launch(lib, src, b, out, v, a, stats=None, bnb=None, ax=None):
    bn = bnb if bnb is not None else _NO_BNB
    mode, y2, c1, c2, c3, rsc, rsh, mki, mko, dst = ax
    return lib.pdt_conv_nt_ax(_p(src), _p(b), _p(out), _p(stats), a["Hs"], a["Ws"], a["Cs"], a["Nimg"], a["Hm"],
                              a["Wm"], a["Ncol"], a["K"], a["ldb"], a["ldo"], int(v), _p(bn[0]), _p(bn[1]),
                              _p(bn[2]), _p(bn[3]), _p(bn[4]), _p(bn[5]), int(bn[6]), int(bn[7]), int(bn[8]),
                              int(mode), _p(y2), _p(c1), _p(c2), _p(c3), _p(rsc), _p(rsh), _p(mki), _p(mko), _p(dst),
                              _s())


def _ax2_launch(lib, src, b, out, v, a, stats=None, bnb=None, ax=None, addend=None, addend_mask=None):
    bn = bnb if bnb is not None else _NO_BNB
    mode, y2, c1, c2, c3, rsc, rsh, mki, mko, dst = ax
    return lib.pdt_conv_nt_ax3(
        _p(src), _p(b), _p(out), _p(stats), _p(addend), _p(addend_mask), a["Hs"], a["Ws"], a["Cs"], a["Nimg"], a["Hm"], a["Wm"], a["Ncol"], a["K"],
        a["ldb"], a["sh"], a["sw"], a["oh0"], a["ow0"], a["dh"], a["dw"], a["nth"], a["ntw"], a["Ho"], a["Wo"],
        a["osh"], a["osw"], a["oph"], a["opw"], a["ldo"], int(v), _p(bn[0]), _p(bn[1]), _p(bn[2]), _p(bn[3]),
        _p(bn[4]), _p(bn[5]), int(bn[6]), int(bn[7]), int(bn[8]), int(mode), _p(y2), _p(c1), _p(c2), _p(c3), _p(rsc),
        _p(rsh), _p(mki), _p(mko), _p(dst), _s())


def _ax_select(key, run, run_ref=None):
    return autotune.choose(key, lambda: (AX_VARIANTS, run), AX_VARIANTS[3],
                           retune="PDT_RETUNE_AX", ref=run_ref)


def _conv3_dgrad_bn_bwd(dout, u3, k1, k2, k3, dy3, u2, side=None):
    N, Cout, H, W = u3.y.shape
    Cin = u3.C
    if u3.g["KH"] != 1 or u3.g["sh"] != 1 or u3.Cs != Cin or Cout % 64 or u2.Cout != Cin or u3.mask is None:
        return None
    lib = _load()
    wt = _DGRAD_W.get(u3.w, Cout, 1, 1, Cin, 0, 0, 1, 1, 1)
    da2 = _empty_cl(N, Cin, H, W, torch.bfloat16, dout.device)
    a = dict(Hs=H, Ws=W, Cs=Cout, Nimg=N, Hm=H, Wm=W, Ncol=Cin, K=Cout, ldb=Cout, ldo=Cin)
    M = N * H * W
    assert u2.y.shape == da2.shape and u2.y.is_contiguous(memory_format=torch.channels_last)
    ax = (2, u3.y, k1, k2, k3, None, None, u3.mask, None, dy3)

    def bnb(part, R):
        return (u2.y, u2.mean, u2.scale, u2.shift, None, part, 1, 0, R)

    def run(v):
        R = lib.pdt_conv_nt_bnb_rows(M, Cin, Cout, v)
        part = torch.empty(2 * R * Cin, dtype=torch.float32, device=dout.device)
        return _ax_launch(lib, dout, wt, da2, v, a, bnb=bnb(part, R), ax=ax)

    def side_apply():
        ud, b1, b2, b3, dyd = side
        _chk(lib.pdt_bn_bwd_apply(_p(dout), _p(ud.y), None, None, None, _p(b1), _p(b2), _p(b3), _p(dyd), None, M,
                                  Cout, 1, _p(u3.mask), _s()), "bn_bwd_apply (shortcut)")

    def run_ref():
        if side is None:
            _chk(lib.pdt_bn_bwd_apply(_p(dout), _p(u3.y), None, None, None, _p(k1), _p(k2), _p(k3), _p(dy3), None,
                                      M, Cout, 1, _p(u3.mask), _s()), "bn_bwd_apply")
        else:
            ud, b1, b2, b3, dyd = side
            _chk(lib.pdt_bn_bwd_apply_dual(_p(dout), _p(u3.mask), _p(u3.y), _p(k1), _p(k2), _p(k3), _p(dy3),
                                           _p(ud.y), _p(b1), _p(b2), _p(b3), _p(dyd), M, Cout, _s()),
                 "bn_bwd_apply_dual")
        _unit_dx(dy3, u3, bnb_unit=u2)

    def run_tuned(v):
        rc = run(v)
        if rc == 0 and side is not None:
            side_apply()
        return rc

    v = _ax_select(autotune.axb_key(H, W, Cout, N, Cin, side is not None), run_tuned, run_ref)
    if v < 0:
        return None
    R = lib.pdt_conv_nt_bnb_rows(M, Cin, Cout, v)
    part = torch.empty(2 * R * Cin + lib.pdt_rows_reduce_workspace(R, Cin), dtype=torch.float32, device=dout.device)
    rc = _ax_launch(lib, dout, wt, da2, v, a, bnb=bnb(part, R), ax=ax)
    if rc == NOT_APPLICABLE:
        return None
    _chk(rc, "conv_nt_ax (bn3 backward apply + conv3 dgrad)")
    if side is not None:
        side_apply()
    return da2, _BnbPartials(part, R, u2)


def _materialize(u: _Unit):
    _apply_pending(u)
    u.pend = None


def _apply_pending(u: _Unit):
    res, ru, out = u.pend
    lib = _load()
    M = u.y.numel() // u.Cout
    if ru is not None:
        _chk(lib.pdt_bn_apply_res_affine(_p(u.y), _p(res), _p(out), _p(u.scale), _p(u.shift), _p(ru.scale),
                                         _p(ru.shift), M, u.Cout, 1, _p(u.mask), _s()), "bn_apply_res_affine")
    else:
        _chk(lib.pdt_bn_apply(_p(u.y), _p(res), _p(out), _p(u.scale), _p(u.shift), M, u.Cout, 1, _p(u.mask), _s()),
             "bn_apply")


def _conv_fwd_ax(pu: _Unit, xbuf, wb, N, H, W, Cs, Cout, g, with_stats):
    res, ru, _ = pu.pend
    Ho, Wo = g["Ho"], g["Wo"]
    M = N * Ho * Wo
    if g["sh"] != 1 or g["sw"] != 1 or Ho != H or Wo != W or Cs != pu.Cout or Cs % 64 or Cout % 8 or \
            N * H * W * Cs >= _AX_MAX_ELEMS or not pu.relu:
        return None
    lib = _load()
    y = _empty_cl(N, Cout, Ho, Wo, torch.bfloat16, xbuf.device)
    a = _fwd_nt_geom(N, H, W, Cs, Cout, g)
    K = a["K"]
    ax = (1, res, pu.scale, pu.shift, None, ru.scale if ru is not None else None,
          ru.shift if ru is not None else None, None, pu.mask, xbuf)

    def stats(v, tail):
        if not with_stats:
            return None, 0
        R = lib.pdt_conv_nt_stat_rows(M, Cout, K, v)
        ws = lib.pdt_rows_reduce_workspace(R, Cout) if tail else 0
        return torch.empty(2 * R * Cout + ws, dtype=torch.float32, device=xbuf.device), R

    def run(v):
        return _ax2_launch(lib, pu.y, wb, y, v, a, stats=stats(v, False)[0], ax=ax)

    def run_ref():
        _apply_pending(pu)
        _conv_forward(xbuf, wb, N, H, W, Cs, Cout, g, with_stats=with_stats)

    key = autotune.axf_key(H, W, Cs, N, Cout, res is not None, ru is not None, with_stats, g["KH"], g["KW"], g["ph"])
    v = _ax_select(key, run, run_ref)
    if v < 0:
        return None
    part, R = stats(v, True)
    rc = _ax2_launch(lib, pu.y, wb, y, v, a, stats=part, ax=ax)
    if rc == NOT_APPLICABLE:
        return None
    _chk(rc, "conv_nt_ax (deferred BN apply + conv)")
    return y, M, part, R


def _conv2_dgrad_bn_bwd(da2, u2, k1, k2, k3, dy2, u1, bnb_mask=None, addend=None, addend_mask=None):
    g = u2.g
    N, Cout, Ho, Wo = u2.y.shape
    Cin = u2.C
    if g["sh"] != 1 or g["sw"] != 1 or Ho != u2.H or Wo != u2.W or u2.Cs != Cin or Cout % 64 or u1.Cout != Cin or \
            u2.mask is not None or not u2.relu or N * Ho * Wo * Cout >= _AX_MAX_ELEMS:
        return None
    KH, KW, ph, pw = g["KH"], g["KW"], g["ph"], g["pw"]
    lib = _load()
    wt = _DGRAD_W.get(u2.w, Cout, KH, KW, Cin, 0, 0, 1, KH, KW)
    da1 = _empty_cl(N, Cin, u2.H, u2.W, torch.bfloat16, da2.device)
    a = dict(Hs=Ho, Ws=Wo, Cs=Cout, Nimg=N, Hm=u2.H, Wm=u2.W, Ncol=Cin, K=KH * KW * Cout, ldb=KH * KW * Cout, sh=1,
             sw=1, oh0=ph, ow0=pw, dh=-1, dw=-1, nth=KH, ntw=KW, Ho=u2.H, Wo=u2.W, osh=1, osw=1, oph=0, opw=0,
             ldo=Cin)
    M = N * u2.H * u2.W
    ax = (3, u2.y, k1, k2, k3, u2.scale, u2.shift, None, None, dy2)
    if addend is not None:
        _check_addend(addend, da1, addend_mask, Cin)
    if bnb_mask is not None:
        assert bnb_mask.dtype == torch.uint8 and bnb_mask.numel() * 8 == da1.numel()

    def bnb(part, R):
        return (u1.y, u1.mean, u1.scale, u1.shift, bnb_mask, part, 1, 0, R)

    def run(v):
        R = lib.pdt_conv_nt_bnb_rows(M, Cin, a["K"], v)
        part = torch.empty(2 * R * Cin, dtype=torch.float32, device=da2.device)
        return _ax2_launch(lib, da2, wt, da1, v, a, bnb=bnb(part, R), ax=ax, addend=addend, addend_mask=addend_mask)

    def run_ref():
        _chk(lib.pdt_bn_bwd_apply(_p(da2), _p(u2.y), None, _p(u2.scale), _p(u2.shift), _p(k1), _p(k2), _p(k3),
                                  _p(dy2), None, N * Ho * Wo, Cout, 1, None, _s()), "bn_bwd_apply")
        _unit_dx(dy2, u2, addend=addend, addend_mask=addend_mask, bnb_unit=u1, bnb_mask=bnb_mask)

    key = autotune.ax3_key(Ho, Wo, Cout, N, Cin, KH, KW, ph, addend is not None, addend_mask is not None,
                           bnb_mask is not None)
    v = _ax_select(key, run, run_ref)
    if v < 0:
        return None
    R = lib.pdt_conv_nt_bnb_rows(M, Cin, a["K"], v)
    part = torch.empty(2 * R * Cin + lib.pdt_rows_reduce_workspace(R, Cin), dtype=torch.float32, device=da2.device)
    rc = _ax2_launch(lib, da2, wt, da1, v, a, bnb=bnb(part, R), ax=ax, addend=addend, addend_mask=addend_mask)
    if rc == NOT_APPLICABLE:
        return None
    _chk(rc, "conv_nt_ax (BN backward apply + conv dgrad)")
    return da1, _BnbPartials(part, R, u1)


def _unit_dw(dy, u: _Unit):
    w = u.w
    KH, KW = u.g["KH"], u.g["KW"]
    if u.Cs == u.C and w.is_contiguous(memory_format=torch.channels_last):
        dw = _grad_buf(w, tuple(w.shape), torch.channels_last)
        _conv_wgrad(dy, u.x, u.N, u.H, u.W, u.Cs, u.Cout, u.g, dw)
    else:
        tmp = torch.empty((u.Cout, u.Cs, KH, KW), dtype=torch.float32, device=dy.device,
                          memory_format=torch.channels_last)
        _conv_wgrad(dy, u.x, u.N, u.H, u.W, u.Cs, u.Cout, u.g, tmp)
        dw = _grad_buf(w, tuple(w.shape), torch.channels_last).copy_(tmp[:, :u.C]) if u.Cs != u.C else tmp
    return dw.to(w.dtype) if dw.dtype != w.dtype else dw


class _ConvBNAct(torch.autograd.Function):
    @staticmethod
    def forward(ctx, x, w, gamma, beta, residual, conv, relu, bna):
        out, u = _unit_fwd(x, w, gamma, beta, residual, conv, relu, bna)
        ctx.u = u
        ctx.save_for_backward(u.x, u.y, u.mask)
        return out

    @staticmethod
    def backward(ctx, dA):
        u = ctx.u
        dy, dres, dgamma, dbeta = _bn_bwd(dA, u, u.has_res)
        dx = _unit_dx(dy, u) if ctx.needs_input_grad[0] else None
        dw = _unit_dw(dy, u) if ctx.needs_input_grad[1] else None
        del ctx.u
        return (dx, dw, dgamma if ctx.needs_input_grad[2] else None, dbeta if ctx.needs_input_grad[3] else None,
                dres, None, None, None)


def conv_bn_act(x, conv: nn.Conv2d, bn: nn.BatchNorm2d, residual=None, relu=True):
    if not supports_conv(x, conv) or (residual is not None and residual.dtype != torch.bfloat16):
        fallback("conv_bn_act", f"conv {tuple(conv.kernel_size)}/{tuple(conv.stride)} groups={conv.groups} "
                                f"bias={conv.bias is not None} on {tuple(x.shape)} {x.dtype}")
        from ..fused import _torch_conv_bn_act
        return _torch_conv_bn_act(x, conv, bn, residual, relu)
    return _ConvBNAct.apply(x, conv.weight, bn.weight, bn.bias, residual, conv, relu, _BNArgs(bn))
```

### pytorch_distributed_template_amd/ops/native_ops/gemm.py

```python
from __future__ import annotations

import ctypes
import os

import torch

from .. import autotune
from .lib import _chk, _load, _p, _s, c_int
from .tuning import AX_UNFUSED, NOT_APPLICABLE


def _nt_args(src, b, out, stats, bias, a, act, variant, addend=None, aux=None, addend_mask=None):
    return (_p(src), _p(b), _p(out), _p(stats), _p(bias), _p(addend), _p(addend_mask), a["Hs"], a["Ws"], a["Cs"], a["Nimg"], a["Hm"], a["Wm"],
            a["Ncol"], a["K"], a["ldb"], a["sh"], a["sw"], a["oh0"], a["ow0"], a["dh"], a["dw"], a["nth"], a["ntw"],
            a["Ho"], a["Wo"], a["osh"], a["osw"], a["oph"], a["opw"], a["ldo"], int(act), _p(aux), int(variant),
            int(a.get("pix", 0)), _s())


_AX_MAX_ELEMS = 2 ** 32 - 8


def _check_nt(src, b, out, a):
    assert src.dtype == torch.bfloat16 and b.dtype == torch.bfloat16 and out.dtype == torch.bfloat16
    Cs, K, Ncol, ldo, ldb = a["Cs"], a["K"], a["Ncol"], a["ldo"], a["ldb"]
    assert Cs % 8 == 0 and K % 8 == 0 and Ncol % 8 == 0 and ldo % 8 == 0, (Cs, K, Ncol, ldo)
    assert K == a["nth"] * a["ntw"] * Cs
    pix = a.get("pix", 0) or Cs
    assert pix % 4 == 0 and pix <= Cs
    assert src.numel() >= a["Nimg"] * a["Hs"] * a["Ws"] * pix, "src too small"
    assert b.numel() >= Ncol * ldb or K == 0, "B too small"
    assert out.numel() >= a["Nimg"] * a["Ho"] * a["Wo"] * ldo, "out too small"
    assert a["Hm"] * a["osh"] <= a["Ho"] and a["Wm"] * a["osw"] <= a["Wo"]
    assert a["Nimg"] * a["Hs"] * a["Ws"] < 2 ** 31 and a["Nimg"] * a["Ho"] * a["Wo"] < 2 ** 31


def select_nt_variant(src, b, out, *, with_stats=False, bias=None, act=0, aux=None, addend=None, **a):
    M, Ncol, K = a["Nimg"] * a["Hm"] * a["Wm"], a["Ncol"], a["K"]

    def setup():
        lib = _load()
        _check_nt(src, b, out, a)
        ids = range(lib.pdt_conv_nt_num_variants())
        rows = max(lib.pdt_conv_nt_stat_rows(M, Ncol, K, v) for v in ids)
        stats = torch.empty(2 * rows * Ncol, dtype=torch.float32, device=src.device) if with_stats else None
        tune_add = addend if act in (3, 5) else None
        return ids, lambda v: lib.pdt_conv_nt(*_nt_args(src, b, out, stats, bias, a, act, v, aux=aux,
                                                        addend=tune_add))

    return autotune.choose(
        autotune.nt_key(a["Hs"], a["Ws"], a["Cs"], a["Nimg"], a["Hm"], a["Wm"], Ncol, K, a["sh"], a["sw"], a["nth"],
                        a["ntw"], a["osh"], with_stats, bias is not None, a.get("pix", 0), act),
        setup, lambda: _load().pdt_conv_nt_resolve_variant(-1, M, Ncol, K),
        retune="PDT_RETUNE_WITH", first_only="PDT_NT_VARIANTS")


ACT = {None: 0, "none": 0, "relu": 1, "gelu": 2}
ACT_GELU_GRAD, ACT_GELU_DUAL, ACT_MUL = 3, 4, 5


def _gelu_dual() -> bool:
    return os.environ.get("PDT_GELU_DUAL", "1") == "1"


def conv_nt(src, b, out, *, stats=None, bias=None, relu=False, act=None, variant=None, addend=None, aux=None,
            addend_mask=None, **a):
    _check_nt(src, b, out, a)
    if addend is not None:
        _check_addend(addend, out, addend_mask, a["Ncol"])
    act_id = (act if isinstance(act, int) else ACT[act]) if act is not None else (1 if relu else 0)
    if aux is not None:
        assert aux.dtype == torch.bfloat16 and aux.numel() == out.numel()
    if variant is None:
        variant = select_nt_variant(src, b, out, with_stats=stats is not None, bias=bias, act=act_id, aux=aux,
                                    addend=addend, **a)
    if addend_mask is not None:
        assert addend is not None and a["ldo"] == a["Ncol"]
    lib = _load()
    rc = lib.pdt_conv_nt(*_nt_args(src, b, out, stats, bias, a, act_id, variant, addend, aux, addend_mask))
    if rc == NOT_APPLICABLE:
        M = a["Nimg"] * a["Hm"] * a["Wm"]
        variant = lib.pdt_conv_nt_resolve_variant(-1, M, a["Ncol"], a["K"])
        rc = lib.pdt_conv_nt(*_nt_args(src, b, out, stats, bias, a, act_id, variant, addend, aux, addend_mask))
    _chk(rc, "conv_nt")


def _check_addend(addend, out, addend_mask, Ncol):
    assert addend.dtype == torch.bfloat16 and addend.numel() == out.numel() and addend.is_contiguous(
        memory_format=torch.channels_last if addend.dim() == 4 else torch.contiguous_format)
    if addend_mask is not None:
        assert addend_mask.dtype == torch.uint8 and addend_mask.numel() * 8 == addend.numel()


def conv_stat_rows(M, Ncol, K, variant):
    return _load().pdt_conv_nt_stat_rows(M, Ncol, K, variant)


def _wgrad_launch(lib, dy, x, out, v, scale, accumulate, a, bias_out=None, bna=None):
    kps = c_int(0)
    splits = lib.pdt_wgrad_plan2(a["M"], a["Mo"], a["No"], a["Hs"], a["Ws"], a["C"], v, ctypes.byref(kps))
    if splits < 0:
        return splits
    slab = torch.empty(lib.pdt_wgrad_workspace(splits, a["Mo"], a["No"]), dtype=torch.float32, device=dy.device)
    by, bc = bna if bna is not None else (None, None)
    return lib.pdt_conv_wgrad2(_p(dy), _p(x), _p(slab), _p(out), a["M"], a["Mo"], a["No"], a["ldy"], a["Hs"],
                               a["Ws"], a["C"], a["Hm"], a["Wm"], a["sh"], a["sw"], a["oh0"], a["ow0"], a["dh"],
                               a["dw"], a["ntw"], splits, kps.value, float(scale), int(accumulate), int(v),
                               int(a.get("pix", 0)), _p(bias_out), _p(by), _p(bc), _s())


WGB_VARIANTS = tuple(range(12))


def conv_wgrad_bn(dA, x, out, y, coef, run_ref, **a):
    lib = _load()
    assert coef.dtype == torch.float32 and coef.is_contiguous() and coef.numel() == 5 * a["Mo"]
    assert y.dtype == torch.bfloat16 and y.shape == dA.shape

    def run(v):
        return _wgrad_launch(lib, dA, x, out, v, 1.0, False, a, bna=(y, coef))

    v = autotune.choose(_wg_key(a, True), lambda: (WGB_VARIANTS, run), AX_UNFUSED, ref=run_ref)
    if v < 0:
        return False
    _chk(run(v), "conv_wgrad (BN backward apply)")
    return True


def _wg_key(a, bn=False):
    return autotune.wg_key(a["M"], a["Mo"], a["No"], a["Hs"], a["Ws"], a["C"], a["Hm"], a["Wm"], a["sh"], a["ntw"],
                           a.get("pix", 0), bn)


def conv_wgrad(dy, x, out, *, scale=1.0, accumulate=False, variant=None, bias_out=None, **a):
    M, Mo, No, ldy, C, Hm, Wm = a["M"], a["Mo"], a["No"], a["ldy"], a["C"], a["Hm"], a["Wm"]
    assert dy.dtype == torch.bfloat16 and x.dtype == torch.bfloat16 and out.dtype == torch.float32
    assert C % 8 == 0 and Mo % 8 == 0 and No % 8 == 0 and ldy % 8 == 0
    assert out.numel() >= Mo * No and dy.numel() >= M * ldy
    pix = a.get("pix", 0) or C
    assert pix % 4 == 0 and pix <= C
    assert M % (Hm * Wm) == 0 and x.numel() >= (M // (Hm * Wm)) * a["Hs"] * a["Ws"] * pix, "wgrad source too small"
    assert a["ntw"] >= 1 and No % C == 0
    if bias_out is not None:
        assert bias_out.dtype == torch.float32 and bias_out.numel() >= Mo and bias_out.is_contiguous()
        assert bias_out.device == dy.device, "bias gradient buffer on another device than dY"
    assert out.device == dy.device == x.device, "weight gradient operands on different devices"
    lib = _load()
    if variant is None:
        variant = autotune.choose(
            _wg_key(a), lambda: (range(lib.pdt_wgrad_num_variants()),
                                 lambda v: _wgrad_launch(lib, dy, x, out, v, scale, False, a)),
            -1, retune="PDT_RETUNE_WG")
    rc = _wgrad_launch(lib, dy, x, out, variant, scale, accumulate, a, bias_out)
    if rc == NOT_APPLICABLE:
        rc = _wgrad_launch(lib, dy, x, out, -1, scale, accumulate, a, bias_out)
    _chk(rc, "conv_wgrad")


def colsum(x, R, C):
    assert x.dtype == torch.bfloat16 and x.numel() >= R * C
    lib = _load()
    out = torch.empty(C, dtype=torch.float32, device=x.device)
    work = torch.empty(lib.pdt_colsum_workspace(R, C), dtype=torch.float32, device=x.device)
    _chk(lib.pdt_colsum(_p(x), _p(out), _p(work), R, C, 0, _s()), "colsum")
    return out
```

Before: 14950 images/sec.

## Recompute BN+ReLU of conv input inside wgrad staging instead of materializing it

Adds an XBN mode to the wgrad kernels (generic and 3x3 halo) that applies the previous layer's BN scale/shift and ReLU to X while staging it into LDS. The forward fused BN-apply+conv path can then skip writing the activated tensor, keeping the pre-BN output plus scale/shift for backward. This removes one activation write in forward and its re-read in backward, at the cost of extra ALU work and an LDS pass per tile in the wgrad kernels. Selection goes through an autotuned pairing and falls back to materializing the tensor when unsupported.

```diff
diff --git a/csrc/conv3x3_halo.hip b/csrc/conv3x3_halo.hip
--- a/csrc/conv3x3_halo.hip
+++ b/csrc/conv3x3_halo.hip
@@ -357,6 +357,8 @@
   const void* zero;
   int M, Mo, C, H, W, rs_log2, ntiles, tps, nco, ncc;
   FastDiv div_H;
+  const float* x_scale;
+  const float* x_shift;
 };
 
 constexpr int HW_DY = HBM * 128;
@@ -369,10 +371,11 @@
           uintptr_t)(smem + byte)));
 }
 
+template <bool XBN>
 __global__ void __launch_bounds__(512, 1) wgrad3x3_halo_kernel(HWParams p) {
   constexpr int NTH = 512, KS = HBM / 32;
   constexpr int LP = PMAX / (NTH / 8);
-  __shared__ __attribute__((aligned(16))) char smem[HW_LDS];
+  __shared__ __attribute__((aligned(16))) char smem[HW_LDS + (XBN ? 512 : 0)];
   const int tid = threadIdx.x, lane = tid & 63, wave = tid >> 6;
   const int wc = wave >> 2, wg = wave & 3;
   const int W = p.W, H = p.H, C = p.C;
@@ -448,10 +451,50 @@
   for (int t = 0; t < 9; ++t) acc[t][0] = acc[t][1] = f32x4{0.f, 0.f, 0.f, 0.f};
   __syncthreads();
 
+  const int xc0 = ((tid & 7) ^ ((tid >> 4) & 7)) << 3;
+  if constexpr (XBN) {
+    float* cf = reinterpret_cast<float*>(smem + HW_LDS);
+    if (tid < 64) cf[tid] = p.x_scale[cc * 64 + tid];
+    else if (tid < 128) cf[tid] = p.x_shift[cc * 64 + tid - 64];
+    __syncthreads();
+  }
+
   if (t_begin < t_end) issue(t_begin, 0);
   for (int tj = t_begin; tj < t_end; ++tj) {
     const int buf = (tj - t_begin) & 1;
     asm volatile("s_waitcnt vmcnt(0)" ::: "memory");
+    if constexpr (XBN) {
+      const int g0 = tj * k - 1;
+      char* sp = smem + buf * PBYTES;
+      float xsc[8], xsh[8];
+      {
+        const f32x4* cf = reinterpret_cast<const f32x4*>(smem + HW_LDS + xc0 * 4);
+        const f32x4 s0 = cf[0], s1 = cf[1], h0 = cf[16], h1 = cf[17];
+#pragma unroll
+        for (int e = 0; e < 4; ++e) { xsc[e] = s0[e]; xsc[4 + e] = s1[e]; xsh[e] = h0[e]; xsh[4 + e] = h1[e]; }
+      }
+#pragma unroll
+      for (int l = 0; l < LP; ++l) {
+        const int qq = (tid >> 3) + (NTH / 8) * l;
+        const int gr = g0 + (qq >> p.rs_log2);
+        const int w = (qq & (rs - 1)) - 1;
+        if (qq < P && gr >= 0 && gr < NH && w >= 0 && w < W) {
+          u32x4* q = reinterpret_cast<u32x4*>(sp + qq * 128 + (tid & 7) * 16);
+          u32x4 v = *q;
+          float f[8];
+#pragma unroll
+          for (int e = 0; e < 4; ++e) { f[2 * e] = lo_bf(v[e]); f[2 * e + 1] = hi_bf(v[e]); }
+#pragma unroll
+          for (int e = 0; e < 8; ++e) f[e] = f[e] * xsc[e] + xsh[e];
+#pragma unroll
+          for (int e = 0; e < 8; ++e) f[e] = fmaxf(f[e], 0.f);
+#pragma unroll
+          for (int e = 0; e < 4; ++e) v[e] = pack2bf(f[2 * e], f[2 * e + 1]);
+          *q = v;
+        }
+      }
+      asm volatile("s_waitcnt lgkmcnt(0)" ::: "memory");
+    }
     __builtin_amdgcn_s_barrier();
     asm volatile("" ::: "memory");
     issue(tj + 1, buf ^ 1);
@@ -529,7 +572,7 @@
 }
 
 int run_halo_wgrad(const void* dy, const void* x, float* slab, int M, int Mo, int C, int Hs, int Ws, int splits,
-                   int tps, hipStream_t st) {
+                   int tps, const float* x_scale, const float* x_shift, hipStream_t st) {
   int s2 = 0, t2 = 0;
   const int rc = halo_wgrad_plan(M, Mo, C, Hs, Ws, &s2, &t2);
   if (rc) return rc;
@@ -549,7 +592,12 @@
   p.nco = Mo / 64;
   p.ncc = C / 64;
   p.div_H = make_fastdiv(Hs);
-  hipLaunchKernelGGL(wgrad3x3_halo_kernel, dim3(p.nco * p.ncc * splits), dim3(512), 0, st, p);
+  p.x_scale = x_scale;
+  p.x_shift = x_shift;
+  if (x_scale != nullptr)
+    hipLaunchKernelGGL(wgrad3x3_halo_kernel<true>, dim3(p.nco * p.ncc * splits), dim3(512), 0, st, p);
+  else
+    hipLaunchKernelGGL(wgrad3x3_halo_kernel<false>, dim3(p.nco * p.ncc * splits), dim3(512), 0, st, p);
   PDT_RETURN_LAUNCH();
 }
 
diff --git a/csrc/conv_nt_kernel.h b/csrc/conv_nt_kernel.h
--- a/csrc/conv_nt_kernel.h
+++ b/csrc/conv_nt_kernel.h
@@ -280,6 +280,6 @@
 int halo_rows(int M);
 int halo_wgrad_plan(int M, int Mo, int C, int Hs, int Ws, int* splits, int* tps);
 int run_halo_wgrad(const void* dy, const void* x, float* slab, int M, int Mo, int C, int Hs, int Ws, int splits,
-                   int tps, hipStream_t st);
-
-}
+                   int tps, const float* x_scale, const float* x_shift, hipStream_t st);
+
+}
diff --git a/csrc/conv_wgrad.hip b/csrc/conv_wgrad.hip
--- a/csrc/conv_wgrad.hip
+++ b/csrc/conv_wgrad.hip
@@ -5,7 +5,7 @@
 namespace pdt_nt {
 int halo_wgrad_plan(int M, int Mo, int C, int Hs, int Ws, int* splits, int* tps);
 int run_halo_wgrad(const void* dy, const void* x, float* slab, int M, int Mo, int C, int Hs, int Ws, int splits,
-                   int tps, hipStream_t st);
+                   int tps, const float* x_scale, const float* x_shift, hipStream_t st);
 }
 
 namespace {
@@ -26,6 +26,8 @@
   float* bslab;
   const u16* bn_y;
   const float* bn_c;
+  const float* x_scale;
+  const float* x_shift;
   FastDiv div_Wm, div_HWm, div_C, div_ntw;
   const void* zero;
 };
@@ -66,9 +68,11 @@
   return r;
 }
 
-template <int BM, int BN, int NSTAGE, int NTH = NT, int WM = 2, int PF = 1, bool BIAS = false, bool BNA = false>
+template <int BM, int BN, int NSTAGE, int NTH = NT, int WM = 2, int PF = 1, bool BIAS = false, bool BNA = false,
+          bool XBN = false>
 __global__ void __launch_bounds__(NTH, NTH == NT ? 2 : 1) wgrad_kernel(WGParams p) {
   static_assert(!BNA || (PF == 1 && !BIAS), "the staged BN-backward apply: single register slot, no bias");
+  static_assert(!XBN || (PF == 1 && !BIAS), "the staged BN+ReLU of X: single register slot, no bias");
   constexpr int WN = NTH / 64 / WM;
   constexpr int RBA = BM * 2;
   constexpr int RBB = BN * 2;
@@ -127,6 +131,15 @@
       csh[e] = p.bn_c[4 * p.Mo + c0 + e];
     }
   }
+  bool rvx[XBN ? NB : 1];
+  float xsc[XBN ? 8 : 1], xsh[XBN ? 8 : 1];
+  if constexpr (XBN) {
+#pragma unroll
+    for (int e = 0; e < 8; ++e) {
+      xsc[e] = p.x_scale[cB_ch + e];
+      xsh[e] = p.x_shift[cB_ch + e];
+    }
+  }
   const bool dobias = BIAS && tn == 0;
   f32x4 bacc[BIAS ? MI : 1];
 #pragma unroll
@@ -157,6 +170,7 @@
       ok = ok && (unsigned)ih < (unsigned)p.Hs && (unsigned)iw < (unsigned)p.Ws;
       rb[i] = *reinterpret_cast<const u32x4*>(
           ok ? (const void*)(p.x + ((size_t)(img * p.Hs + ih) * p.Ws + iw) * p.pix + cB_ch) : p.zero);
+      if constexpr (XBN) rvx[i] = ok;
     }
   };
   auto load_tile = [&](int kt) { load_into(kt, ra, rb); };
@@ -184,8 +198,21 @@
       *reinterpret_cast<u32x4*>(sa + lds_off<RBA>(rA0 + AROWS * i, cA * 16)) = v;
     }
 #pragma unroll
-    for (int i = 0; i < NB; ++i)
-      *reinterpret_cast<u32x4*>(sb + lds_off<RBB>(rB0 + BROWS * i, cB * 16)) = rb[i];
+    for (int i = 0; i < NB; ++i) {
+      u32x4 v = rb[i];
+      if constexpr (XBN) {
+        float f[8];
+#pragma unroll
+        for (int e = 0; e < 4; ++e) { f[2 * e] = lo_bf(v[e]); f[2 * e + 1] = hi_bf(v[e]); }
+#pragma unroll
+        for (int k = 0; k < 8; ++k) f[k] = f[k] * xsc[k] + xsh[k];
+#pragma unroll
+        for (int k = 0; k < 8; ++k) f[k] = fmaxf(f[k], 0.f);
+#pragma unroll
+        for (int e = 0; e < 4; ++e) v[e] = rvx[i] ? pack2bf(f[2 * e], f[2 * e + 1]) : 0u;
+      }
+      *reinterpret_cast<u32x4*>(sb + lds_off<RBB>(rB0 + BROWS * i, cB * 16)) = v;
+    }
   };
 
   f32x4 acc[MI][NI];
@@ -390,8 +417,9 @@
   return (nk + kps - 1) / kps;
 }
 
+template <bool BNA, bool XBN>
 static void launch_wg_bna(const WGVar& w, dim3 grid, const WGParams& p, hipStream_t stream) {
-#define WG_LAUNCH_B(a, b, c) hipLaunchKernelGGL((wgrad_kernel<a, b, c, NT, 2, 1, false, true>), grid, dim3(NT), 0, stream, p)
+#define WG_LAUNCH_B(a, b, c) hipLaunchKernelGGL((wgrad_kernel<a, b, c, NT, 2, 1, false, BNA, XBN>), grid, dim3(NT), 0, stream, p)
   if (w.NS == 2) {
     if (w.BM == 64 && w.BN == 64) WG_LAUNCH_B(64, 64, 2);
     else if (w.BM == 64) WG_LAUNCH_B(64, 128, 2);
@@ -404,6 +432,14 @@
     else WG_LAUNCH_B(128, 128, 1);
   }
 #undef WG_LAUNCH_B
+}
+
+static void launch_wg_x8(const WGVar& w, dim3 grid, const WGParams& p, hipStream_t stream) {
+#define WG_LAUNCH_X8(a, b, wm) \
+  hipLaunchKernelGGL((wgrad_kernel<a, b, 2, 512, wm, 1, false, false, true>), grid, dim3(512), 0, stream, p)
+  if (w.BM == 256) WG_LAUNCH_X8(256, 128, 4);
+  else WG_LAUNCH_X8(128, 256, 2);
+#undef WG_LAUNCH_X8
 }
 
 template <bool BIAS>
@@ -560,20 +596,35 @@
                             int dh, int dw, int ntw, int splits, int ktiles_per_split, float scale,
                             int accumulate, int variant, int pix, float* bias_out, const void* bn_y,
                             const float* bn_c, hipStream_t stream) {
+  return pdt_conv_wgrad2x(dy, x, slab, out, M, Mo, No, ldy, Hs, Ws, C, Hm, Wm, sh, sw, oh0, ow0, dh, dw, ntw, splits,
+                          ktiles_per_split, scale, accumulate, variant, pix, bias_out, bn_y, bn_c, nullptr, nullptr,
+                          stream);
+}
+
+PDT_API int pdt_conv_wgrad2x(const void* dy, const void* x, float* slab, float* out, int M, int Mo, int No,
+                             int ldy, int Hs, int Ws, int C, int Hm, int Wm, int sh, int sw, int oh0, int ow0,
+                             int dh, int dw, int ntw, int splits, int ktiles_per_split, float scale,
+                             int accumulate, int variant, int pix, float* bias_out, const void* bn_y,
+                             const float* bn_c, const float* x_scale, const float* x_shift, hipStream_t stream) {
   if (C % 8 != 0 || Mo % 8 != 0 || No % 8 != 0 || ldy % 8 != 0) return -1;
   const bool bna = bn_y != nullptr;
   if (bna && (bn_c == nullptr || variant < 0 || variant >= 12 || bias_out != nullptr)) return -5;
+  const bool xbn = x_scale != nullptr;
+  if (xbn && (x_shift == nullptr || bias_out != nullptr || (pix != 0 && pix != C) ||
+              (variant >= 16 && variant < WG_NVAR) || variant == WG_RING))
+    return -5;
   if (pix != 0 && (pix % 4 != 0 || pix > C)) return -10;
   if (variant == WG_NVAR) {
     if (ntw != 3 || No != 9 * C || sh != 1 || sw != 1 || oh0 != -1 || ow0 != -1 || dh != 1 || dw != 1 ||
         Hm != Hs || Wm != Ws || (pix != 0 && pix != C) || ldy != Mo || bias_out != nullptr || M % Wm != 0)
       return -5;
-    const int rc = pdt_nt::run_halo_wgrad(dy, x, slab, M, Mo, C, Hs, Ws, splits, ktiles_per_split, stream);
+    const int rc = pdt_nt::run_halo_wgrad(dy, x, slab, M, Mo, C, Hs, Ws, splits, ktiles_per_split, x_scale, x_shift,
+                                          stream);
     if (rc) return rc;
     return pdt_wgrad_reduce(slab, out, nullptr, nullptr, splits, Mo, No, scale, accumulate, stream);
   }
   if (variant == WG_RING) {
-    if (bna || bias_out != nullptr) return -5;
+    if (bna || xbn || bias_out != nullptr) return -5;
     const int rc = pdt_wgrad_ring_launch(dy, x, slab, M, Mo, No, ldy, Hs, Ws, C, Hm, Wm, sh, sw, oh0, ow0, dh, dw, ntw,
                                          splits, ktiles_per_split, pix, stream);
     if (rc) return rc;
@@ -590,6 +641,8 @@
   p.ktiles_per_split = ktiles_per_split; p.splits = splits;
   p.bn_y = (const u16*)bn_y;
   p.bn_c = bn_c;
+  p.x_scale = x_scale;
+  p.x_shift = x_shift;
   const int G = reduce_groups(splits, Mo, No);
   p.bslab = bias_out ? slab + (long)splits * Mo * No + (G > 1 ? (long)G * Mo * No : 0) : nullptr;
   static const int xcd_env = pdt_env_flag("PDT_WGRAD_XCD", 1);
@@ -606,7 +659,10 @@
   const WGVar w = wg_variant(variant, Mo, No);
   int tiles = ((Mo + w.BM - 1) / w.BM) * ((No + w.BN - 1) / w.BN);
   dim3 grid(tiles * splits);
-  if (bna) launch_wg_bna(w, grid, p, stream);
+  if (xbn && w.NTH == 512) launch_wg_x8(w, grid, p, stream);
+  else if (xbn && bna) launch_wg_bna<true, true>(w, grid, p, stream);
+  else if (xbn) launch_wg_bna<false, true>(w, grid, p, stream);
+  else if (bna) launch_wg_bna<true, false>(w, grid, p, stream);
   else if (bias_out) launch_wg<true>(w, grid, p, stream);
   else launch_wg<false>(w, grid, p, stream);
   int e = (int)hipGetLastError();
diff --git a/csrc/pdt_api.h b/csrc/pdt_api.h
--- a/csrc/pdt_api.h
+++ b/csrc/pdt_api.h
@@ -125,6 +125,11 @@
                             int Hs, int Ws, int C, int Hm, int Wm, int sh, int sw, int oh0, int ow0, int dh, int dw,
                             int ntw, int splits, int ktiles_per_split, float scale, int accumulate, int variant,
                             int pix, float* bias_out, const void* bn_y, const float* bn_c, hipStream_t stream);
+PDT_API int pdt_conv_wgrad2x(const void* dy, const void* x, float* slab, float* out, int M, int Mo, int No, int ldy,
+                             int Hs, int Ws, int C, int Hm, int Wm, int sh, int sw, int oh0, int ow0, int dh, int dw,
+                             int ntw, int splits, int ktiles_per_split, float scale, int accumulate, int variant,
+                             int pix, float* bias_out, const void* bn_y, const float* bn_c, const float* x_scale,
+                             const float* x_shift, hipStream_t stream);
 PDT_API long pdt_reduce_rows_work(int nrows, int n);
 PDT_API int pdt_wgrad_reduce_rows(const float* rows, float* out, int nrows, int n, float scale, int accumulate,
                                   float* work, hipStream_t stream);
diff --git a/pytorch_distributed_template_amd/ops/autotune.py b/pytorch_distributed_template_amd/ops/autotune.py
--- a/pytorch_distributed_template_amd/ops/autotune.py
+++ b/pytorch_distributed_template_amd/ops/autotune.py
@@ -178,6 +178,11 @@
         (f",k{KH}x{KW}p{ph}" if KH != 1 or KW != 1 else "")
 
 
+@lru_cache(maxsize=None)
+def xwf_key(H, W, Cs, N, Cout, with_stats, KH=1, KW=1, ph=0) -> str:
+    return "xwf:" + _csv(H, W, Cs, N, Cout, int(with_stats)) + (f",k{KH}x{KW}p{ph}" if KH != 1 or KW != 1 else "")
+
+
 def axb_key(H, W, Cout, N, Cin, side=False) -> str:
     return ("axd:" if side else "axb:") + _csv(H, W, Cout, N, Cin)
 
diff --git a/pytorch_distributed_template_amd/ops/native_ops/bn_unit.py b/pytorch_distributed_template_amd/ops/native_ops/bn_unit.py
--- a/pytorch_distributed_template_amd/ops/native_ops/bn_unit.py
+++ b/pytorch_distributed_template_amd/ops/native_ops/bn_unit.py
@@ -1,6 +1,8 @@
 from __future__ import annotations
 
+import ctypes
 import os
+from ctypes import c_int
 
 import torch
 import torch.nn as nn
@@ -8,7 +10,7 @@
 from .. import autotune
 from .conv import (_BnbPartials, _DGRAD_W, _conv_dgrad, _conv_forward, _conv_wgrad, _fwd_geom, _fwd_nt_geom,
                    supports_conv)
-from .gemm import _AX_MAX_ELEMS, _check_addend
+from .gemm import _AX_MAX_ELEMS, _check_addend, conv_wgrad_x, select_nt_variant
 from .lib import _chk, _cl, _empty_cl, _grad_buf, _load, _p, _s, fallback
 from .shadows import bf16_weight
 from .tuning import NOT_APPLICABLE
@@ -35,7 +37,7 @@
 
 
 class _Unit:
-    __slots__ = ("x", "w", "gamma", "beta", "y", "act", "mask", "mean", "invstd", "scale", "shift", "N", "C", "Cs", "H",
+    __slots__ = ("x", "xsrc", "w", "gamma", "beta", "y", "act", "mask", "mean", "invstd", "scale", "shift", "N", "C", "Cs", "H",
                  "W", "Cout", "g", "relu", "has_res", "bnb_pre", "pend", "res_unit", "__weakref__")
 
 
@@ -68,12 +70,14 @@
     wb = bf16_weight(w, pad_cin_to=Cs if Cs != C else None)
     f32 = dict(dtype=torch.float32, device=x.device)
     M = N * g["Ho"] * g["Wo"]
-    r = None
+    r = xsrc = None
     if src_pend is not None and getattr(src_pend, "pend", None) is not None:
         assert src_pend.y.shape == x.shape and x.data_ptr() == src_pend.pend[2].data_ptr()
-        r = _conv_fwd_ax(src_pend, x, wb, N, H, W, Cs, Cout, g, bna.training)
+        r, wrote = _conv_fwd_ax(src_pend, x, wb, N, H, W, Cs, Cout, g, bna.training)
         if r is None:
             _materialize(src_pend)
+        elif not wrote:
+            xsrc = src_pend
         src_pend.pend = None
     if r is None:
         r = _conv_forward(x, wb, N, H, W, Cs, Cout, g, with_stats=bna.training)
@@ -92,7 +96,8 @@
     assert y.numel() == M * Cout
     if not apply:
         u = _Unit()
-        u.x, u.w, u.gamma, u.beta, u.y = x, w, gamma, beta, y
+        u.x, u.w, u.gamma, u.beta, u.y = (x if xsrc is None else None), w, gamma, beta, y
+        u.xsrc = xsrc
         u.act, u.mask, u.bnb_pre, u.pend, u.res_unit = None, None, None, None, None
         u.mean, u.invstd, u.scale, u.shift = mean, invstd, scale, shift
         u.N, u.C, u.Cs, u.H, u.W, u.Cout, u.g, u.relu, u.has_res = N, C, Cs, H, W, Cout, g, relu, False
@@ -116,7 +121,8 @@
     else:
         _chk(lib.pdt_bn_apply(_p(y), _p(res), _p(out), _p(scale), _p(shift), M, Cout, int(relu), _p(mask), st),
              "bn_apply")
-    u.x, u.w, u.gamma, u.beta, u.y = x, w, gamma, beta, y
+    u.x, u.w, u.gamma, u.beta, u.y = (x if xsrc is None else None), w, gamma, beta, y
+    u.xsrc = xsrc
     u.act = None
     u.mask = mask
     u.res_unit = res_unit
@@ -201,6 +207,10 @@
     return os.environ.get("PDT_FUSE_BN_AX", "1") != "0"
 
 
+def _xw_mode() -> int:
+    return int(os.environ.get("PDT_FUSE_BN_XW", "1") or 0)
+
+
 def _conv1_fold_enabled() -> bool:
     return os.environ.get("PDT_FUSE_BN_AX1", "1") != "0"
 
@@ -314,7 +324,7 @@
     M = N * Ho * Wo
     if g["sh"] != 1 or g["sw"] != 1 or Ho != H or Wo != W or Cs != pu.Cout or Cs % 64 or Cout % 8 or \
             N * H * W * Cs >= _AX_MAX_ELEMS or not pu.relu:
-        return None
+        return None, True
     lib = _load()
     y = _empty_cl(N, Cout, Ho, Wo, torch.bfloat16, xbuf.device)
     a = _fwd_nt_geom(N, H, W, Cs, Cout, g)
@@ -337,15 +347,64 @@
         _conv_forward(xbuf, wb, N, H, W, Cs, Cout, g, with_stats=with_stats)
 
     key = autotune.axf_key(H, W, Cs, N, Cout, res is not None, ru is not None, with_stats, g["KH"], g["KW"], g["ph"])
-    v = _ax_select(key, run, run_ref)
+    v0 = _ax_select(key, run, run_ref)
+    xw = _xw_mode() if (res is None and pu.mask is None) else 0
+    if xw:
+        axn = ax[:-1] + (None,)
+        wa = _wgrad_geom(N, H, W, Cs, Cout, g)
+        dws = []
+
+        vp = v0 if v0 >= 0 else select_nt_variant(xbuf, wb, y, with_stats=with_stats, **a)
+
+        def setup():
+            dws.append(torch.empty(Cout * K, dtype=torch.float32, device=xbuf.device))
+
+            def run_pair(v):
+                rc = _ax2_launch(lib, pu.y, wb, y, v, a, stats=stats(v, False)[0], ax=axn)
+                return rc or conv_wgrad_x(y, pu.y, pu.scale, pu.shift, dws[0], **wa)
+
+            return ((vp,) if vp in AX_VARIANTS else ()), run_pair
+
+        def ref_pair():
+            if not dws:
+                dws.append(torch.empty(Cout * K, dtype=torch.float32, device=xbuf.device))
+            if v0 < 0 or run(v0) == NOT_APPLICABLE:
+                run_ref()
+            _conv_wgrad(y, xbuf, N, H, W, Cs, Cout, g, dws[0])
+
+        if xw == 2:
+            vx = vp if vp in AX_VARIANTS else -1
+        else:
+            vx = autotune.choose(autotune.xwf_key(H, W, Cs, N, Cout, with_stats, g["KH"], g["KW"], g["ph"]), setup,
+                                 autotune.AX_UNFUSED, ref=ref_pair, ref_first=True)
+        if vx >= 0 and vx == vp and _wgrad_x_ok(lib, wa):
+            part, R = stats(vx, True)
+            rc = _ax2_launch(lib, pu.y, wb, y, vx, a, stats=part, ax=axn)
+            if rc != NOT_APPLICABLE:
+                _chk(rc, "conv_nt_ax (BN apply without write-back + conv)")
+                return (y, M, part, R), False
+    v = v0
     if v < 0:
-        return None
+        return None, True
     part, R = stats(v, True)
     rc = _ax2_launch(lib, pu.y, wb, y, v, a, stats=part, ax=ax)
     if rc == NOT_APPLICABLE:
-        return None
+        return None, True
     _chk(rc, "conv_nt_ax (deferred BN apply + conv)")
-    return y, M, part, R
+    return (y, M, part, R), True
+
+
+def _wgrad_geom(N, H, W, Cs, Cout, g):
+    return dict(M=N * g["Ho"] * g["Wo"], Mo=Cout, No=g["KH"] * g["KW"] * Cs, ldy=Cout, Hs=H, Ws=W, C=Cs, Hm=g["Ho"],
+                Wm=g["Wo"], sh=g["sh"], sw=g["sw"], oh0=-g["ph"], ow0=-g["pw"], dh=1, dw=1, ntw=g["KW"])
+
+
+def _wgrad_x_ok(lib, wa) -> bool:
+    v = int(autotune.tuned().get(autotune.wg_key(wa["M"], wa["Mo"], wa["No"], wa["Hs"], wa["Ws"], wa["C"], wa["Hm"],
+                                                 wa["Wm"], wa["sh"], wa["ntw"], 0, False), -1))
+    if v == lib.pdt_wgrad_halo_id():
+        return lib.pdt_wgrad_plan2(wa["M"], wa["Mo"], wa["No"], wa["Hs"], wa["Ws"], wa["C"], v, ctypes.byref(c_int(0))) >= 0
+    return v < 16 or v > lib.pdt_wgrad_halo_id() + 1
 
 
 def _conv2_dgrad_bn_bwd(da2, u2, k1, k2, k3, dy2, u1, bnb_mask=None, addend=None, addend_mask=None):
@@ -396,16 +455,29 @@
     return da1, _BnbPartials(part, R, u1)
 
 
+def _unit_wgrad(dy, u: _Unit, out):
+    if u.x is not None:
+        return _conv_wgrad(dy, u.x, u.N, u.H, u.W, u.Cs, u.Cout, u.g, out)
+    p = u.xsrc
+    rc = conv_wgrad_x(dy, p.y, p.scale, p.shift, out, **_wgrad_geom(u.N, u.H, u.W, u.Cs, u.Cout, u.g))
+    if rc == NOT_APPLICABLE:
+        x = torch.empty_like(p.y, memory_format=torch.channels_last)
+        _chk(_load().pdt_bn_apply(_p(p.y), None, _p(x), _p(p.scale), _p(p.shift), p.y.numel() // p.Cout, p.Cout, 1,
+                                  None, _s()), "bn_apply")
+        return _conv_wgrad(dy, x, u.N, u.H, u.W, u.Cs, u.Cout, u.g, out)
+    _chk(rc, "conv_wgrad (BN apply in the X staging)")
+
+
 def _unit_dw(dy, u: _Unit):
     w = u.w
     KH, KW = u.g["KH"], u.g["KW"]
     if u.Cs == u.C and w.is_contiguous(memory_format=torch.channels_last):
         dw = _grad_buf(w, tuple(w.shape), torch.channels_last)
-        _conv_wgrad(dy, u.x, u.N, u.H, u.W, u.Cs, u.Cout, u.g, dw)
+        _unit_wgrad(dy, u, dw)
     else:
         tmp = torch.empty((u.Cout, u.Cs, KH, KW), dtype=torch.float32, device=dy.device,
                           memory_format=torch.channels_last)
-        _conv_wgrad(dy, u.x, u.N, u.H, u.W, u.Cs, u.Cout, u.g, tmp)
+        _unit_wgrad(dy, u, tmp)
         dw = _grad_buf(w, tuple(w.shape), torch.channels_last).copy_(tmp[:, :u.C]) if u.Cs != u.C else tmp
     return dw.to(w.dtype) if dw.dtype != w.dtype else dw
 
diff --git a/pytorch_distributed_template_amd/ops/native_ops/gemm.py b/pytorch_distributed_template_amd/ops/native_ops/gemm.py
--- a/pytorch_distributed_template_amd/ops/native_ops/gemm.py
+++ b/pytorch_distributed_template_amd/ops/native_ops/gemm.py
@@ -95,17 +95,19 @@
     return _load().pdt_conv_nt_stat_rows(M, Ncol, K, variant)
 
 
-def _wgrad_launch(lib, dy, x, out, v, scale, accumulate, a, bias_out=None, bna=None):
+def _wgrad_launch(lib, dy, x, out, v, scale, accumulate, a, bias_out=None, bna=None, xbn=None):
     kps = c_int(0)
     splits = lib.pdt_wgrad_plan2(a["M"], a["Mo"], a["No"], a["Hs"], a["Ws"], a["C"], v, ctypes.byref(kps))
     if splits < 0:
         return splits
     slab = torch.empty(lib.pdt_wgrad_workspace(splits, a["Mo"], a["No"]), dtype=torch.float32, device=dy.device)
     by, bc = bna if bna is not None else (None, None)
-    return lib.pdt_conv_wgrad2(_p(dy), _p(x), _p(slab), _p(out), a["M"], a["Mo"], a["No"], a["ldy"], a["Hs"],
-                               a["Ws"], a["C"], a["Hm"], a["Wm"], a["sh"], a["sw"], a["oh0"], a["ow0"], a["dh"],
-                               a["dw"], a["ntw"], splits, kps.value, float(scale), int(accumulate), int(v),
-                               int(a.get("pix", 0)), _p(bias_out), _p(by), _p(bc), _s())
+    args = (_p(dy), _p(x), _p(slab), _p(out), a["M"], a["Mo"], a["No"], a["ldy"], a["Hs"], a["Ws"], a["C"], a["Hm"],
+            a["Wm"], a["sh"], a["sw"], a["oh0"], a["ow0"], a["dh"], a["dw"], a["ntw"], splits, kps.value,
+            float(scale), int(accumulate), int(v), int(a.get("pix", 0)), _p(bias_out), _p(by), _p(bc))
+    if xbn is not None:
+        return lib.pdt_conv_wgrad2x(*args, _p(xbn[0]), _p(xbn[1]), _s())
+    return lib.pdt_conv_wgrad2(*args, _s())
 
 
 WGB_VARIANTS = tuple(range(12))
@@ -156,6 +158,21 @@
     _chk(rc, "conv_wgrad")
 
 
+def conv_wgrad_x(dy, y, x_scale, x_shift, out, **a):
+    assert dy.dtype == torch.bfloat16 and y.dtype == torch.bfloat16 and out.dtype == torch.float32
+    assert x_scale.dtype == torch.float32 and x_shift.dtype == torch.float32
+    assert x_scale.numel() >= a["C"] and x_shift.numel() >= a["C"] and not a.get("pix", 0)
+    assert out.numel() >= a["Mo"] * a["No"] and dy.numel() >= a["M"] * a["ldy"]
+    assert y.numel() >= (a["M"] // (a["Hm"] * a["Wm"])) * a["Hs"] * a["Ws"] * a["C"], "wgrad source too small"
+    assert out.device == dy.device == y.device, "weight gradient operands on different devices"
+    lib = _load()
+    variant = autotune.choose(
+        _wg_key(a), lambda: (range(lib.pdt_wgrad_num_variants()),
+                             lambda v: _wgrad_launch(lib, dy, y, out, v, 1.0, False, a)),
+        -1, retune="PDT_RETUNE_WG")
+    return _wgrad_launch(lib, dy, y, out, variant, 1.0, False, a, xbn=(x_scale, x_shift))
+
+
 def colsum(x, R, C):
     assert x.dtype == torch.bfloat16 and x.numel() >= R * C
     lib = _load()
```

Result: no change. 14970 images/sec, median of 3 (+0.1%).
